# GenomicBreeding/GenomicBreedingModels.jl

Measured on AMD Instinct MI355X. Metric: GRM+GBLUP genotype-cells/s (n x p), higher is better.
Workload: dtype f64

## Files before the change

genomicbreedingmodels.jl_amd/csrc/capi.cpp:

```cpp
#include <cmath>

#include "fit_ctx.h"

namespace gbm {

static thread_local std::string g_last_error;

void set_error(const std::string& msg) { g_last_error = msg; }
int fail(int code, const std::string& msg) {
  g_last_error = msg;
  return code;
}
const std::string& last_error() { return g_last_error; }

int resolve_grm_mode(int grm_mode) {
  if (grm_mode != GBM_GRM_DEFAULT && grm_mode != GBM_GRM_DROPIN) return grm_mode;
  const char* e = ::gbm::knob("GBM_GRM");
  if (e && strcmp(e, "exact") == 0) return GBM_GRM_EXACT;
  if (e && strcmp(e, "auto") == 0) return GBM_GRM_AUTO;
  if (e && strcmp(e, "fp64") == 0) return GBM_GRM_FP64;
  return grm_mode == GBM_GRM_DROPIN ? GBM_GRM_AUTO : GBM_GRM_FP64;
}

namespace {

int solve_effects(const Problem& pr, Shards& shards, const std::vector<int>& leaders,
                  const std::vector<int>& ldevs, int64_t q, const double* Y, int64_t ldy, int64_t t0, int64_t nt,
                  double lambda, double* b_hat_out, double* y_pred_out, double* mu_out) {
  const int64_t n = pr.n, p = pr.p, npad = npad_of(n), gdim = gdim_of(n);
  const double inv_q = 1.0 / (double)q;
  const bool distributed = (leaders.size() > 1 || force_rccl()) && n >= knob_i64("GBM_DIST_SOLVE_MIN_N", 16384);
  std::vector<int32_t> infos(shards.size(), 0);
  {
    RoctxRange rsolve(distributed ? "gbm: distributed solve" : "gbm: solve");
    for (size_t k = 0; k < shards.size(); k++) {
      Shard& sh = *shards[k];
      FitCtx& c = sh.x();
      GBM_HIP_TRY(hipSetDevice(c.dev));
      hipStream_t s = c.stream.s;
      GBM_TRY(ensure(c.A, c.dev, nt * npad * 8));
      GBM_TRY(ensure(c.B, c.dev, nt * sh.p * 8));
      GBM_TRY(ensure(c.msum, c.dev, nt * 8));
      if (sh.leader != (int)k) continue;
      GBM_TRY(ensure(c.Y, c.dev, nt * npad * 8));
      GBM_TRY(ensure(c.gebv, c.dev, nt * npad * 8));
      GBM_TRY(ensure(c.mu, c.dev, nt * 8));
      GBM_TRY(ensure(c.info, c.dev, 4));
      const int64_t wss = gbm_dev_solve_workspace(n, nt);
      GBM_TRY(ensure(c.wss, c.dev, wss));
      GBM_HIP_TRY(hipMemcpy2DAsync(c.Y.p, npad * 8, Y + t0 * ldy, ldy * 8, n * 8, nt, hipMemcpyHostToDevice, s));
      if (!distributed)
        GBM_TRY(gbm_dev_gblup_solve((double*)c.G.p, gdim, n, inv_q, nullptr, lambda, (const double*)c.Y.p, npad, nt,
                                    (double*)c.A.p, (double*)c.gebv.p, npad, (double*)c.mu.p, (int32_t*)c.info.p,
                                    c.wss.p, wss, s));
    }
    if (distributed) GBM_TRY(solve_distributed(shards, leaders, ldevs, n, inv_q, lambda, nt));
    for (int k : leaders) {
      FitCtx& c = shards[k]->x();
      GBM_HIP_TRY(hipSetDevice(c.dev));
      GBM_HIP_TRY(hipMemcpyAsync(&infos[k], c.info.p, 4, hipMemcpyDeviceToHost, c.stream.s));
    }
    for (int k : leaders) {
      FitCtx& c = shards[k]->x();
      GBM_HIP_TRY(hipSetDevice(c.dev));
      GBM_HIP_TRY(hipStreamSynchronize(c.stream.s));
      const int32_t info = infos[k];
      if (info < 0) return fail(GBM_E_HIP, "solve: a wait between workgroups timed out (dataflow Cholesky or back substitution; the result is invalid)");
      if (info != 0)
        return fail(GBM_E_NOTPD, "G/q + lambda*I is not positive definite (pivot " + std::to_string(info) +
                                     "); check for non-finite genotypes");
    }
  }
  RoctxRange reff("gbm: marker effects + download");
  std::vector<std::vector<double>> msums(shards.size(), std::vector<double>(nt, 0.0));
  std::vector<double> mu(nt, 0.0);
  double* bo = b_hat_out + t0 * (p + 1);
  for (size_t k = 0; k < shards.size(); k++) {
    Shard& sh = *shards[k];
    FitCtx& c = sh.x();
    GBM_HIP_TRY(hipSetDevice(c.dev));
    hipStream_t s = c.stream.s;
    if (sh.leader != (int)k)
      GBM_HIP_TRY(hipMemcpyAsync(c.A.p, shards[sh.leader]->x().A.p, nt * npad * 8, hipMemcpyDeviceToDevice, s));
    if (sh.stream || sh.exact)
      GBM_TRY(stream_effects_shard(pr, sh, nt, inv_q));
    else
      GBM_TRY(gbm_dev_marker_effects((const double*)c.Xt.p, npad, sh.p, n, (const double*)c.A.p, npad, nt, inv_q,
                                     nullptr, (const double*)c.mean.p, (const double*)c.sd.p, (const int32_t*)c.keep.p,
                                     (double*)c.B.p, sh.p, (double*)c.msum.p, s));
    GBM_HIP_TRY(hipMemcpy2DAsync(bo + 1 + sh.j0, (p + 1) * 8, c.B.p, sh.p * 8, sh.p * 8, nt, hipMemcpyDeviceToHost, s));
    GBM_HIP_TRY(hipMemcpyAsync(msums[k].data(), c.msum.p, nt * 8, hipMemcpyDeviceToHost, s));
    if (k == 0) {
      GBM_HIP_TRY(hipMemcpy2DAsync(y_pred_out + t0 * n, n * 8, c.gebv.p, npad * 8, n * 8, nt, hipMemcpyDeviceToHost, s));
      GBM_HIP_TRY(hipMemcpyAsync(mu.data(), c.mu.p, nt * 8, hipMemcpyDeviceToHost, s));
    }
  }
  std::vector<double> msum_total(nt, 0.0);
  for (size_t k = 0; k < shards.size(); k++) {
    GBM_HIP_TRY(hipSetDevice(shards[k]->x().dev));
    GBM_HIP_TRY(hipStreamSynchronize(shards[k]->x().stream.s));
    for (int64_t t = 0; t < nt; t++) msum_total[t] += msums[k][t];
  }
  for (int64_t t = 0; t < nt; t++) {
    bo[t * (p + 1)] = mu[t] - msum_total[t];
    if (mu_out) mu_out[t0 + t] = mu[t];
  }
  return GBM_OK;
}

struct RemlOut {
  double* lambda;
  double* s2e;
  double* s2u;
};

int reml_lambda(FitCtx& c, int64_t n, int64_t q, const double* y, RemlResult& res) {
  const int64_t npad = npad_of(n), gdim = gdim_of(n);
  GBM_HIP_TRY(hipSetDevice(c.dev));
  hipStream_t s = c.stream.s;
  const int64_t wss = gbm_dev_solve_workspace(n, 1);
  GBM_TRY(ensure(c.Y, c.dev, npad * 8));
  GBM_TRY(ensure(c.A, c.dev, npad * 8));
  GBM_TRY(ensure(c.gebv, c.dev, npad * 8));
  GBM_TRY(ensure(c.mu, c.dev, 8));
  GBM_TRY(ensure(c.info, c.dev, 4));
  GBM_TRY(ensure(c.wss, c.dev, wss));
  GBM_TRY(ensure(c.tmp, c.dev, 4 * 8));
  const std::vector<double> ys = standardise_y(y, n);
  GBM_HIP_TRY(hipMemsetAsync(c.Y.p, 0, (size_t)(npad * 8), s));
  GBM_HIP_TRY(hipMemcpyAsync(c.Y.p, ys.data(), n * 8, hipMemcpyHostToDevice, s));
  auto eval = [&](double lambda, RemlEval& e) -> int {
    GBM_HIP_TRY(hipMemcpyAsync(c.G.p, c.Gc.p, (size_t)(npad * gdim * 8), hipMemcpyDeviceToDevice, s));
    GBM_TRY(gbm_dev_gblup_solve((double*)c.G.p, gdim, n, 1.0 / (double)q, nullptr, lambda, (const double*)c.Y.p, npad,
                                1, (double*)c.A.p, (double*)c.gebv.p, npad, (double*)c.mu.p, (int32_t*)c.info.p, c.wss.p,
                                wss, s));
    GBM_TRY(gbm_dev_gblup_terms((const double*)c.G.p, gdim, n, 1, c.wss.p, (double*)c.tmp.p, s));
    double t[4];
    int32_t info = 0;
    GBM_HIP_TRY(hipMemcpyAsync(t, c.tmp.p, 4 * 8, hipMemcpyDeviceToHost, s));
    GBM_HIP_TRY(hipMemcpyAsync(&info, c.info.p, 4, hipMemcpyDeviceToHost, s));
    GBM_HIP_TRY(hipStreamSynchronize(s));
    if (info < 0) return fail(GBM_E_HIP, "solve: a wait between workgroups timed out (dataflow Cholesky or back substitution; the result is invalid)");
    if (info != 0) return fail(GBM_E_NOTPD, "REML: G/q + lambda*I is not positive definite (pivot " + std::to_string(info) + ")");
    e = reml_profile(n, lambda, t);
    return GBM_OK;
  };
  return reml_search(eval, res);
}

int run_fit(const Problem& pr, const double* Y, int64_t ldy, int64_t nrhs, double lambda, const int* devices, int ndev,
            double* b_hat_out, double* y_pred_out, double* mu_out, int64_t* q_out, const RemlOut* reml = nullptr,
            int grm_mode = GBM_GRM_DEFAULT, int* grm_used_out = nullptr) {
  const int64_t n = pr.n, p = pr.p;
  if (n < 2) return fail(GBM_E_DATA, "there are less than 2 entries (reference src/prediction.jl:117-123)");
  if (p < 1 || pr.ld < n || !Y || ldy < n || nrhs < 1 || nrhs > 63 || !b_hat_out || !y_pred_out)
    return fail(GBM_E_ARG, "gbm_gblup_fit: bad arguments (need p >= 1, ldx >= n, ldy >= n, 1 <= nrhs <= 63, outputs)");
  if (!reml && (!(lambda > 0.0) || !std::isfinite(lambda)))
    return fail(GBM_E_ARG, "gbm_gblup_fit: lambda must be finite and > 0");
  if (reml && n < 3) return fail(GBM_E_DATA, "REML needs at least 3 entries");
  GBM_TRY(check_y(Y, n, ldy, nrhs));
  const int mode = resolve_grm_mode(grm_mode);
  if (mode != GBM_GRM_FP64 && mode != GBM_GRM_EXACT && mode != GBM_GRM_AUTO)
    return fail(GBM_E_ARG, "grm_mode must be GBM_GRM_DEFAULT, GBM_GRM_FP64, GBM_GRM_EXACT or GBM_GRM_AUTO (GBM_GRM: fp64 | exact | auto)");
  if (mode == GBM_GRM_EXACT && pr.src == Source::I8 && pr.ploidy != 2)
    return fail(GBM_E_ARG, "grm_mode exact: the exact-integer GRM needs diploid dosages (ploidy 2)");
  std::vector<int> devs;
  GBM_TRY(check_devices(devices, ndev, devs));
  const int64_t npad = npad_of(n), gdim = gdim_of(n);
  Shards shards;
  GBM_TRY(make_shards(devs, p, shards));
  int64_t q = 0, pmax = 0;
  for (auto& sh : shards) pmax = std::max(pmax, sh->p);
  const int64_t chunk = pr.src == Source::SYNTH ? 0 : host_chunk(pmax);
  bool exact = mode != GBM_GRM_FP64 && !(pr.src == Source::I8 && pr.ploidy != 2);
  const bool host_pack = knob_i64("GBM_HOST_PACK", 1) != 0;
  const int pack_threads = std::max(1, host_pack_threads() / (int)shards.size());
  auto fp64_grm = [&]() -> int {
    GBM_TRY(plan_streaming(pr, shards, reml != nullptr));
    const bool pack = mode == GBM_GRM_FP64 && pr.src == Source::F64 && host_pack;
    return parallel_shards(shards, [&](size_t, Shard& sh) {
      if (sh.stream) return stream_grm_shard(pr, sh);
      if (chunk > 0) {
        if (pack) {
          const int rc = upload_grm_pipelined_packed(pr, sh, chunk, pack_threads);
          if (rc != kNotDosage) return rc;
        }
        return upload_grm_pipelined(pr, sh, chunk);
      }
      return prepare_grm_shard(pr, sh);
    });
  };
  {
    RoctxRange r("gbm: upload + standardise + GRM");
    if (exact) {
      for (auto& sh : shards) sh->exact = true;
      const int rc = parallel_shards(shards, [&](size_t, Shard& sh) {
        if (pr.src == Source::F64) {
          if (host_pack)
            GBM_TRY(host_pack_upload_shard(pr, sh, pack_threads));
          else
            GBM_TRY(dosage_upload_shard(pr, sh, mode == GBM_GRM_AUTO));
        }
        return exact_grm_shard(pr, sh, mode == GBM_GRM_AUTO && pr.src == Source::I8);
      });
      if (rc == kNotDosage && mode == GBM_GRM_EXACT)
        return fail(GBM_E_ARG, "grm_mode exact: the genotypes are not diploid dosages (2x must be exactly 0, 1 or 2 "
                               "in every cell; use grm_mode auto or fp64)");
      const bool fallback = mode == GBM_GRM_AUTO && (rc == kNotDosage || rc == GBM_E_OOM || rc == GBM_E_ARG);
      if (fallback) {
        exact = false;
        for (auto& sh : shards) {
          sh->exact = sh->d8_ready = false;
          FitCtx& c = sh->x();
          if (pr.src == Source::F64 && c.D8.p) {
            (void)hipSetDevice(c.dev);
            c.D8.reset();
            c.D8.cap = 0;
          }
        }
        set_error("");
      } else {
        GBM_TRY(rc);
      }
    }
    if (!exact) GBM_TRY(fp64_grm());
  }
  if (grm_used_out) *grm_used_out = exact ? GBM_GRM_EXACT : GBM_GRM_FP64;
  for (auto& sh : shards) q += sh->q_host;
  if (q_out) *q_out = q;
  if (q == 0) return fail(GBM_E_DATA, "no polymorphic locus-allele (all standard deviations <= eps, src/gwas.jl:112-115)");
  {
    RoctxRange r("gbm: partial-GRM all-reduce");
    GBM_TRY(allreduce_grm(shards, n));
  }
  std::vector<int> leaders, ldevs;
  shard_leaders(shards, leaders, ldevs);
  if (!reml) return solve_effects(pr, shards, leaders, ldevs, q, Y, ldy, 0, nrhs, lambda, b_hat_out, y_pred_out, mu_out);
  const int64_t vbytes = npad * gdim * 8;
  FitCtx& c0 = shards[leaders[0]]->x();
  GBM_HIP_TRY(hipSetDevice(c0.dev));
  GBM_TRY(ensure(c0.Gc, c0.dev, gdim * gdim * 8));
  GBM_HIP_TRY(hipMemcpyAsync(c0.Gc.p, c0.G.p, (size_t)vbytes, hipMemcpyDeviceToDevice, c0.stream.s));
  std::vector<double> lam(nrhs);
  {
    RoctxRange r("gbm: REML lambda");
    for (int64_t t = 0; t < nrhs; t++) {
      RemlResult res;
      GBM_TRY(reml_lambda(shards[leaders[0]]->x(), n, q, Y + t * ldy, res));
      lam[t] = res.lambda;
      if (reml->lambda) reml->lambda[t] = res.lambda;
      if (reml->s2e) reml->s2e[t] = res.s2e;
      if (reml->s2u) reml->s2u[t] = res.s2u;
    }
  }
  GBM_HIP_TRY(hipSetDevice(c0.dev));
  GBM_HIP_TRY(hipStreamSynchronize(c0.stream.s));
  for (int64_t t = 0; t < nrhs; t++) {
    for (int k : leaders) {
      FitCtx& c = shards[k]->x();
      GBM_TRY(copy_dd(c, c.G.p, c0, c0.Gc.p, vbytes));
    }
    GBM_TRY(solve_effects(pr, shards, leaders, ldevs, q, Y, ldy, t, 1, lam[t], b_hat_out, y_pred_out, mu_out));
  }
  return GBM_OK;
}

int export_grm(FitCtx& c, int64_t n, double scale, double* G_out, int64_t ldg) {
  GBM_HIP_TRY(hipSetDevice(c.dev));
  GBM_TRY(ensure(c.out, c.dev, n * n * 8));
  GBM_TRY(launch_grm_export((const double*)c.G.p, gdim_of(n), n, scale, (double*)c.out.p, n, c.stream.s));
  GBM_HIP_TRY(hipMemcpy2DAsync(G_out, ldg * 8, c.out.p, n * 8, n * 8, n, hipMemcpyDeviceToHost, c.stream.s));
  GBM_HIP_TRY(hipStreamSynchronize(c.stream.s));
// ... 234 lines not shown
```

genomicbreedingmodels.jl_amd/csrc/chol.hip:

```cpp
#include <cstdlib>
#include <string>

#include "chol_device.h"

namespace gbm {

constexpr int NB = kCholNB;
constexpr int MAXRHS = 63;

int launch_chol_update(double* G, int64_t ldg, int64_t k0, int64_t nb, int64_t gdim, double* Ld, double* Dinv,
                       int32_t* info, int64_t next_k0, int rank, int nranks, hipStream_t s, int64_t col_lo = 0,
                       int64_t col_hi = INT64_MAX, int64_t row_lo = 0, int64_t row_hi = INT64_MAX);
int launch_chol_row_update(double* G, int64_t ldg, int64_t k0, int kch, int64_t gdim, double* Ld, double* Dinv,
                           int32_t* info, hipStream_t s, ColKeep keep = ColKeep{});
int64_t chol_small_lim();
void chol_refresh_tuning();
int64_t chol_flow_flag_bytes(int64_t gdim);
bool chol_flow_enabled(int64_t npad);
int launch_chol_flow(double* G, int64_t ldg, int64_t gdim, double* Ld, double* Dinv, void* flag_block, int32_t* info,
                     hipStream_t s);

__global__ void __launch_bounds__(256) prepare_v_kernel(double* __restrict__ G, int64_t ld, int64_t n,
                                                        int64_t npad, int64_t gdim, double inv_q,
                                                        const int64_t* __restrict__ q_dev, double lambda,
                                                        const double* __restrict__ Y, int64_t ldy, int64_t nrhs,
                                                        int32_t* __restrict__ info, ColKeep keep) {
  const int64_t i = blockIdx.x;
  if (i == 0 && threadIdx.x == 0) *info = 0;
  if (q_dev) inv_q = 1.0 / (double)(*q_dev);
  double* row = G + i * ld;
  const int64_t jbeg = (i / NB) * NB;
  for (int64_t j = jbeg + threadIdx.x; j < gdim; j += 256) {
    if (keep.nranks > 1 && !col_kept(keep, j)) continue;
    double v = 0.0;
    if (i < npad) {
      if (j < i) v = 0.0;
      else if (j < npad) v = (i < n && j < n) ? row[j] * inv_q + (i == j ? lambda : 0.0) : (i == j ? 1.0 : 0.0);
      else if (i < n) {
        const int64_t t = j - npad;
        v = t == 0 ? 1.0 : (t <= nrhs ? Y[(t - 1) * ldy + i] : 0.0);
      }
    }
    row[j] = v;
  }
}

__global__ void __launch_bounds__(256) factor_diag_kernel(const double* __restrict__ G, int64_t ld, int64_t k,
                                                          double* __restrict__ Ld, double* __restrict__ Dinv,
                                                          int32_t* __restrict__ info) {
  __shared__ __attribute__((aligned(16))) double Us[CNB * PS];
  __shared__ double rinv[CNB + 16];
  const int tid = threadIdx.x;
  {
    const int row = tid >> 2, quarter = tid & 3;
    const double* sa = G + (k + row) * ld + k + quarter * 16;
#pragma unroll
    for (int e = 0; e < 16; e += 2)
      *reinterpret_cast<double2*>(&Us[row * PS + quarter * 16 + e]) = *reinterpret_cast<const double2*>(sa + e);
  }
  __syncthreads();
  const int bad = factor_diag_block(Us, rinv, tid);
  if (tid == 0 && bad >= 0) atomicCAS(info, 0, (int32_t)(k + bad + 1));
  store_factor(Us, rinv, Ld + k * CNB, Dinv + (k / 16) * 256, tid);
}

__global__ void __launch_bounds__(256) chol_strip_kernel(double* __restrict__ G, int64_t ld, int64_t r0,
                                                         int64_t rows, int64_t J0, int64_t Jend, int64_t cnt,
                                                         int owner, int nranks, double* __restrict__ buf,
                                                         int unpack) {
  const int src = unpack ? (int)blockIdx.z : owner;
  const int64_t m = blockIdx.y;
  const int64_t row = (int64_t)blockIdx.x * 4 + (threadIdx.x >> 6);
  const int c2 = threadIdx.x & 63;
  if (row >= rows) return;
  const int64_t r = (m * rows + row) * 64 + c2;
  double2* b2 = reinterpret_cast<double2*>(buf) + (unpack ? (int64_t)src * cnt * rows * 64 + r : r);
  const int j0 = (int)J0;
  const int64_t J = J0 + ((src - j0) % nranks + nranks) % nranks + m * nranks;
  if (J >= Jend) {
    if (!unpack) *b2 = make_double2(0.0, 0.0);
    return;
  }
  double2* g2 = reinterpret_cast<double2*>(G + (r0 + row) * ld + J * 128) + c2;
  if (unpack)
    *g2 = *b2;
  else
    *b2 = *g2;
}

__global__ void __launch_bounds__(256) chol_panel_kernel(double* __restrict__ G, int64_t ld, int64_t k0,
                                                         const double* __restrict__ Ld,
                                                         const double* __restrict__ Dinv, ColKeep keep) {
  __shared__ __attribute__((aligned(16))) double Us[CNB * PS];
  __shared__ __attribute__((aligned(16))) double X[CNB * PS];
  __shared__ __attribute__((aligned(16))) double Di[4 * 256];
  const int tid = threadIdx.x, lane = tid & 63, wave = tid >> 6;
  const int64_t jx = k0 + ((int64_t)blockIdx.x + 1) * CNB;
  if (!col_kept(keep, jx)) return;
  const int lrow = tid >> 5, lcol = 2 * (tid & 31);
  {
    const double* sl = Ld + (k0 + lrow) * CNB + lcol;
    const double* sx = G + (k0 + lrow) * ld + jx + lcol;
    double2 vl[8], vx[8];
// ... 251 lines not shown
      *reinterpret_cast<double2*>(G + (jx + row) * ld + r0 + lcol) = make_double2(X[lcol * PS + row], X[(lcol + 1) * PS + row]);
    }
    if (area) {
#pragma unroll
      for (int ks = 0; ks < 16; ks++) {
        double af[2], bf[2];
#pragma unroll
        for (int m = 0; m < 2; m++) af[m] = -X[(ks * 4 + fr) * PS + wm * 32 + m * 16 + fc];
#pragma unroll
        for (int q = 0; q < 2; q++) bf[q] = X[(ks * 4 + fr) * PS + wn * 32 + q * 16 + fc];
#pragma unroll
        for (int m = 0; m < 2; m++)
#pragma unroll
          for (int q = 0; q < 2; q++) accd[m][q] = __builtin_amdgcn_mfma_f64_16x16x4f64(af[m], bf[q], accd[m][q], 0, 0, 0);
      }
      publish_flag(&prog[c], j + 1, tid);
    } else {
      __syncthreads();
    }
  }
}

__global__ void __launch_bounds__(64) diag_inverse_kernel(const double* __restrict__ Ld, double* __restrict__ Linv) {
  __shared__ double Ub[NB][NB + 1];
  const int lane = threadIdx.x;
  const int64_t b0 = (int64_t)blockIdx.x * NB;
  for (int r = 0; r < NB; r++) Ub[r][lane] = Ld[(b0 + r) * NB + lane];
  __syncthreads();
  double x[NB];
#pragma unroll
  for (int i = NB - 1; i >= 0; i--) {
    double p0 = 0.0, p1 = 0.0, p2 = 0.0, p3 = 0.0;
#pragma unroll
    for (int k = i + 1; k < NB; k += 4) {
      p0 = fma(Ub[i][k], x[k], p0);
      if (k + 1 < NB) p1 = fma(Ub[i][k + 1], x[k + 1], p1);
      if (k + 2 < NB) p2 = fma(Ub[i][k + 2], x[k + 2], p2);
      if (k + 3 < NB) p3 = fma(Ub[i][k + 3], x[k + 3], p3);
    }
    x[i] = (i <= lane) ? (((lane == i) ? 1.0 : 0.0) - ((p0 + p1) + (p2 + p3))) * rcp_nr(Ub[i][i]) : 0.0;
  }
#pragma unroll
  for (int i = 0; i < NB; i++) Linv[(b0 + i) * NB + lane] = x[i];
}

__global__ void __launch_bounds__(256) gls_mu_kernel(const double* __restrict__ G, int64_t ld, int64_t npad,
                                                     int64_t nrhs, double* __restrict__ W, int64_t lda,
                                                     double* __restrict__ mu, int32_t* __restrict__ flags) {
  const int64_t t = blockIdx.y;
  const double c11 = -G[npad * ld + npad];
  const double c1y = -G[npad * ld + npad + 1 + t];
  const double m = c1y / c11;
  if (blockIdx.x == 0 && threadIdx.x == 0) mu[t] = m;
  if (t == 0)
    for (int64_t i = (int64_t)blockIdx.x * 256 + threadIdx.x; i < npad / NB; i += (int64_t)gridDim.x * 256) flags[i] = 0;
  for (int64_t i = (int64_t)blockIdx.x * 256 + threadIdx.x; i < lda; i += (int64_t)gridDim.x * 256)
    W[t * lda + i] = i < npad ? G[(npad + 1 + t) * ld + i] - m * G[npad * ld + i] : 0.0;
}

__global__ void __launch_bounds__(256) gblup_terms_kernel(const double* __restrict__ G, int64_t ld, int64_t npad,
                                                          int64_t nrhs, const double* __restrict__ Ld,
                                                          double* __restrict__ terms) {
  __shared__ double red[256];
  double sacc = 0.0;
  for (int64_t r = threadIdx.x; r < npad; r += 256) sacc += log(Ld[r * NB + (r % NB)]);
  red[threadIdx.x] = sacc;
  __syncthreads();
  for (int w = 128; w > 0; w >>= 1) {
    if ((int)threadIdx.x < w) red[threadIdx.x] += red[threadIdx.x + w];
    __syncthreads();
  }
  if (threadIdx.x == 0) {
    terms[0] = 2.0 * red[0];
    terms[1] = -G[npad * ld + npad];
  }
  for (int64_t t = threadIdx.x; t < nrhs; t += 256) {
    terms[2 + 2 * t] = -G[npad * ld + npad + 1 + t];
    terms[3 + 2 * t] = -G[(npad + 1 + t) * ld + npad + 1 + t];
  }
}

constexpr int RC = 4;

__global__ void __launch_bounds__(256) back_solve_kernel(const double* __restrict__ G, int64_t ld,
                                                         const double* __restrict__ Linv, int64_t nb,
                                                         const double* __restrict__ W, double* A,
                                                         int64_t lda, int64_t nrhs, int32_t* __restrict__ flags,
                                                         int32_t* __restrict__ info) {
  __shared__ double part[4][RC][NB];
  __shared__ double rl[RC][NB];
  __shared__ double ah[RC][NB];
  __shared__ int ok_s;
  const int tid = threadIdx.x, lane = tid & 63, wave = tid >> 6;
  const int64_t bh = nb - 1 - 2 * (int64_t)blockIdx.x, bl = bh - 1;
  const bool lo = bl >= 0;
  const int64_t h0 = bh * NB, l0 = bl * NB;
  const int j0 = wave * 16;
  const int64_t a_bytes = nrhs * lda * 8;
  const __amdgpu_buffer_rsrc_t rA =
      __builtin_amdgcn_make_buffer_rsrc(A, (short)0, (int)(a_bytes < 0x7fffffff ? a_bytes : 0x7fffffff), 0x00020000);
  double uh[16], ul[16], lb[16];
#pragma unroll
  for (int jj = 0; jj < 16; jj++) {
    uh[jj] = Linv[(h0 + lane) * NB + j0 + jj];
    ul[jj] = lo ? Linv[(l0 + lane) * NB + j0 + jj] : 0.0;
    lb[jj] = lo ? G[(h0 + j0 + jj) * ld + l0 + lane] : 0.0;
  }
  if (tid == 0) ok_s = 1;
  int32_t pass = 0;
  auto solve_block = [&](int64_t b0, const double (&ui)[16], const double (&acc)[RC], const double (&w)[RC], int tc,
                         int64_t t0, double (*out)[NB]) {
#pragma unroll
    for (int t = 0; t < RC; t++) part[wave][t][lane] = acc[t];
    lds_sync();
    if (wave == 0)
#pragma unroll
      for (int t = 0; t < RC; t++)
        if (t < tc) rl[t][lane] = w[t] - (((part[0][t][lane] + part[1][t][lane]) + part[2][t][lane]) + part[3][t][lane]);
    lds_sync();
    for (int t = 0; t < tc; t++) {
      double s = 0.0;
#pragma unroll
      for (int jj = 0; jj < 16; jj++) s = fma(ui[jj], rl[t][j0 + jj], s);
      part[wave][t][lane] = s;
    }
    lds_sync();
    if (wave == 0)
      for (int t = 0; t < tc; t++) {
        const double v = ((part[0][t][lane] + part[1][t][lane]) + part[2][t][lane]) + part[3][t][lane];
        st_agent(A + (t0 + t) * lda + b0 + lane, v);
        if (out) out[t][lane] = v;
      }
  };
  for (int64_t t0 = 0; t0 < nrhs; t0 += RC) {
    pass++;
    const int tc = (int)(nrhs - t0 < RC ? nrhs - t0 : RC);
    double acch[RC] = {0.0, 0.0, 0.0, 0.0}, accl[RC] = {0.0, 0.0, 0.0, 0.0};
    double wh[RC] = {0.0, 0.0, 0.0, 0.0}, wl[RC] = {0.0, 0.0, 0.0, 0.0};
    if (wave == 0)
#pragma unroll
      for (int t = 0; t < RC; t++)
        if (t < tc) {
          wh[t] = W[(t0 + t) * lda + h0 + lane];
          if (lo) wl[t] = W[(t0 + t) * lda + l0 + lane];
        }
    bool ok = true;
    for (int64_t c = nb - 1; c > bh && ok; c--) {
      double lh[16], ll[16];
      const double* lp = G + (c * NB + j0) * ld + lane;
#pragma unroll
      for (int jj = 0; jj < 16; jj++) {
        lh[jj] = lp[(int64_t)jj * ld + h0];
        ll[jj] = lo ? lp[(int64_t)jj * ld + l0] : 0.0;
      }
      if (lane == 0) ok = wait_flag<false>(&flags[c], pass, info);
      ok = __builtin_amdgcn_readfirstlane((int)ok) != 0;
      __builtin_amdgcn_fence(__ATOMIC_ACQUIRE, "wavefront");
      for (int t = 0; t < tc; t++) {
        const uint32_t voff = (uint32_t)(((t0 + t) * lda + c * NB + j0) * 8);
        double av[16];
#pragma unroll
        for (int jj = 0; jj < 16; jj++)
          av[jj] = __builtin_bit_cast(double, __builtin_amdgcn_raw_buffer_load_b64(rA, (int)(voff + jj * 8), 0, 16));
        double sh = 0.0, sl = 0.0;
#pragma unroll
        for (int jj = 0; jj < 16; jj++) {
          sh = fma(lh[jj], av[jj], sh);
          sl = fma(ll[jj], av[jj], sl);
        }
        acch[t] += sh;
        accl[t] += sl;
      }
    }
    if (!ok) ok_s = 0;
    solve_block(h0, uh, acch, wh, tc, t0, lo ? ah : nullptr);
    publish_flag(&flags[bh], pass, tid);
    if (lo) {
      for (int t = 0; t < tc; t++) {
        double sl = 0.0;
#pragma unroll
        for (int jj = 0; jj < 16; jj++) sl = fma(lb[jj], ah[t][j0 + jj], sl);
        accl[t] += sl;
      }
      lds_sync();
      solve_block(l0, ul, accl, wl, tc, t0, nullptr);
      publish_flag(&flags[bl], pass, tid);
    }
    if (!ok_s) return;
    lds_sync();
  }
}

constexpr int WPA = CNB + 4;
__global__ void __launch_bounds__(512) whiten_rows_kernel(const double* __restrict__ G, int64_t ldg,
                                                          const double* __restrict__ Linv, int64_t nb, double* R,
                                                          int64_t ldr, int64_t rows) {
  __shared__ __attribute__((aligned(16))) double As[2][CNB * WPA];
  __shared__ __attribute__((aligned(16))) double Bs[2][CNB * PS];
  const int tid = threadIdx.x, lane = tid & 63, wave = tid >> 6;
  const int wm = wave >> 2, wn = wave & 3, fr = lane >> 4, fc = lane & 15;
  const int64_t r0 = (int64_t)blockIdx.x * CNB;
  const int lrow = tid >> 5, lcol = 2 * (tid & 31);
  const int cw = wn * 16 + fc;
  typedef double d8 __attribute__((ext_vector_type(8)));
  for (int64_t k = 0; k < nb; k++) {
    d4 acc[2];
#pragma unroll
    for (int m = 0; m < 2; m++)
#pragma unroll
      for (int r = 0; r < 4; r++) {
        const int64_t row = r0 + wm * 32 + m * 16 + fr + 4 * r;
        acc[m][r] = row < rows ? R[row * ldr + k * CNB + cw] : 0.0;
      }
    d8 va0, vb0, va1, vb1;
    auto load_step = [&](int64_t m, d8& va, d8& vb) {
#pragma unroll
      for (int e = 0; e < 4; e++) {
        const int64_t row = r0 + lrow + 16 * e;
        double2 x = make_double2(0.0, 0.0);
        if (row < rows) x = *reinterpret_cast<const double2*>(R + row * ldr + m * CNB + lcol);
        const double2 y = *reinterpret_cast<const double2*>(G + (m * CNB + lrow + 16 * e) * ldg + k * CNB + lcol);
        va[2 * e] = x.x;
        va[2 * e + 1] = x.y;
        vb[2 * e] = y.x;
        vb[2 * e + 1] = y.y;
      }
    };
    auto stage = [&](int buf, const d8& va, const d8& vb) {
#pragma unroll
      for (int e = 0; e < 4; e++) {
        *reinterpret_cast<double2*>(&As[buf][(lrow + 16 * e) * WPA + lcol]) = make_double2(va[2 * e], va[2 * e + 1]);
        *reinterpret_cast<double2*>(&Bs[buf][(lrow + 16 * e) * PS + lcol]) = make_double2(vb[2 * e], vb[2 * e + 1]);
      }
    };
    auto step = [&](int64_t m, int buf, d8& na, d8& nb_) {
      const double* Am = As[buf];
      const double* Bm = Bs[buf];
#pragma unroll
      for (int ks = 0; ks < 16; ks++) {
        const double bf = Bm[(ks * 4 + fr) * PS + cw];
#pragma unroll
        for (int mm = 0; mm < 2; mm++) {
          const double af = -Am[(wm * 32 + mm * 16 + fc) * WPA + ks * 4 + fr];
          acc[mm] = __builtin_amdgcn_mfma_f64_16x16x4f64(af, bf, acc[mm], 0, 0, 0);
        }
      }
      if (m + 1 < k) {
        stage(buf ^ 1, na, nb_);
        if (m + 3 < k) load_step(m + 3, na, nb_);
      }
      __syncthreads();
    };
    if (k > 0) {
      load_step(0, va0, vb0);
      if (k > 1) load_step(1, va1, vb1);
      stage(0, va0, vb0);
      if (k > 2) load_step(2, va0, vb0);
      __syncthreads();
    }
    for (int64_t m = 0; m < k; m += 2) {
      step(m, 0, va1, vb1);
      if (m + 1 < k) step(m + 1, 1, va0, vb0);
    }
#pragma unroll
    for (int m = 0; m < 2; m++)
#pragma unroll
      for (int r = 0; r < 4; r++) As[0][(wm * 32 + m * 16 + fr + 4 * r) * WPA + cw] = acc[m][r];
#pragma unroll
// ... 18 lines not shown
#pragma unroll
      for (int r = 0; r < 4; r++) {
        const int64_t row = r0 + wm * 32 + m * 16 + fr + 4 * r;
        if (row < rows) R[row * ldr + k * CNB + cw] = out[m][r];
      }
    __builtin_amdgcn_s_waitcnt(0);
    __syncthreads();
  }
}

__global__ void __launch_bounds__(256) gebv_kernel(const double* __restrict__ Y, int64_t ldy, int64_t n,
                                                   const double* __restrict__ A, double* __restrict__ gebv,
                                                   int64_t lda, const double* __restrict__ mu, double lambda) {
  const int64_t t = blockIdx.y;
  const double m = mu[t];
  for (int64_t i = (int64_t)blockIdx.x * 256 + threadIdx.x; i < lda; i += (int64_t)gridDim.x * 256)
    gebv[t * lda + i] = i < n ? m + (Y[t * ldy + i] - m) - lambda * A[t * lda + i] : 0.0;
}

}

using namespace gbm;

extern "C" int64_t gbm_dev_npad(int64_t n) { return npad_of(n); }
extern "C" int64_t gbm_dev_gdim(int64_t n) { return gdim_of(n); }
static int64_t flow_block_offset(int64_t n) { return round_up(npad_of(n) * (2 * NB + 16) + npad_of(n) / NB / 2 + 1, 2); }
static int64_t solve_ws_doubles(int64_t n) { return flow_block_offset(n) + chol_flow_flag_bytes(gdim_of(n)) / 8; }
extern "C" int64_t gbm_dev_solve_workspace(int64_t n, int64_t nrhs) {
  (void)nrhs;
  return solve_ws_doubles(n) * (int64_t)sizeof(double);
}

namespace {

struct SolveWs {
  double *Ld, *Linv, *Dinv;
  int32_t* flags;
  void* flow;
};
SolveWs solve_ws(void* workspace, int64_t npad) {
  SolveWs w;
  w.Ld = (double*)workspace;
  w.Linv = w.Ld + npad * NB;
  w.Dinv = w.Linv + npad * NB;
  w.flags = reinterpret_cast<int32_t*>(w.Dinv + npad * 16);
  w.flow = (double*)workspace + flow_block_offset(npad);
  return w;
}

int check_solve_args(const double* G, int64_t ldg, int64_t n, const int32_t* info, const void* workspace,
                     int64_t ws_bytes, const char* who) {
  if (!G || !info || n < 1 || ldg < gdim_of(n) || (ldg & 1) || ((uintptr_t)G & 15))
    return fail(GBM_E_ARG, std::string(who) + ": bad arguments (G 16-byte aligned, even ldg >= gdim(n))");
  if (!workspace || ws_bytes < solve_ws_doubles(n) * (int64_t)sizeof(double) || ((uintptr_t)workspace & 15))
    return fail(GBM_E_ARG, std::string(who) + ": workspace too small (see gbm_dev_solve_workspace)");
  return GBM_OK;
}

static int64_t tail_flow_rows(int64_t npad) {
  const char* e = ::gbm::knob("GBM_CHOL_TAIL_FLOW");
  if (e) return (int64_t)atoll(e);
  return npad > 12288 ? 8192 : 0;
}
static bool tail_flow_at(int64_t kb, int64_t npad, int64_t gdim) {
  return kb > 0 && kb < npad / NB && gdim - kb * NB <= tail_flow_rows(npad);
}

int group_size(int64_t kb, int64_t nb, int64_t gdim) {
  if (tail_flow_at(kb, nb * NB, gdim)) return (int)(nb - kb);
  auto lim = [](const char* name, int64_t dflt) {
    const char* e = ::gbm::knob(name);
    return e ? (int64_t)atoll(e) : dflt;
  };
  const int64_t g4 = lim("GBM_CHOL_G4_LIM", 8192), g8 = lim("GBM_CHOL_G8_LIM", 8192),
                g16 = lim("GBM_CHOL_G16_LIM", 16384);
  const int64_t k0 = kb * NB;
  if (g16 >= 0 && kb + 16 < nb && gdim - (k0 + 16 * NB) > g16) return 16;
  if (g8 >= 0 && kb + 8 < nb && gdim - (k0 + 8 * NB) > g8) return 8;
  if (g4 >= 0 && kb + 4 < nb && gdim - (k0 + 4 * NB) > g4) return 4;
  if (kb + 2 < nb && gdim - (k0 + 2 * NB) > chol_small_lim()) return 2;
  return 1;
}

int solve_prepare(double* G, int64_t ldg, int64_t n, double inv_q, const int64_t* q_dev, double lambda,
                  const double* Y, int64_t ldy, int64_t nrhs, int32_t* info, void* workspace, hipStream_t s,
                  bool factor_first = true, ColKeep keep = ColKeep{}) {
  const int64_t npad = npad_of(n), gdim = gdim_of(n);
  const SolveWs w = solve_ws(workspace, npad);
  chol_refresh_tuning();
  prepare_v_kernel<<<(unsigned)gdim, 256, 0, s>>>(G, ldg, n, npad, gdim, inv_q, q_dev, lambda, Y, ldy, nrhs, info,
                                                  keep);
  GBM_LAUNCH_CHECK();
  if (!factor_first) return GBM_OK;
  factor_diag_kernel<<<1, 256, 0, s>>>(G, ldg, 0, w.Ld, w.Dinv, info);
  GBM_LAUNCH_CHECK();
  return GBM_OK;
}

static bool group_kernel_enabled() {
  const char* e = ::gbm::knob("GBM_CHOL_GROUP_KERNEL");
  return !e || atoi(e) != 0;
}

int solve_group_panels(double* G, int64_t ldg, int64_t n, int64_t kb, ColKeep keep, int32_t* info, void* workspace,
                       hipStream_t s, int64_t* g_out) {
  const int64_t npad = npad_of(n), gdim = gdim_of(n), nb = npad / NB;
  const SolveWs w = solve_ws(workspace, npad);
  const int64_t k0 = kb * NB;
  if (tail_flow_at(kb, npad, gdim))
    return fail(GBM_E_ARG, "gbm_dev_chol_group_panels: the dataflow tail (GBM_CHOL_TAIL_FLOW) runs as gbm_dev_chol_group");
  const int g = group_size(kb, nb, gdim);
  if (keep.nranks > 1) {
    if (g < 2 || (k0 % 128) != 0)
      return fail(GBM_E_ARG, "gbm_dev_chol_group_panels: a distributed step needs a panel group of >= 2 panels on a "
                             "128-row boundary (finish the tail with gbm_dev_chol_group, nranks = 1)");
    keep.keep_hi = k0 + g * NB;
    keep.rhs0 = npad;
  }
  if (g_out) *g_out = g;
  if (g > 1 && group_kernel_enabled()) {
    GroupCols gc;
    gc.g = g;
    gc.nranks = keep.nranks;
    gc.a0 = kb + g;
    gc.rhs0 = npad / NB;
    gc.n_rhs = (gdim - npad) / NB;
    if (keep.nranks == 1) {
      gc.n_own = npad / NB - gc.a0;
    } else {
      const int64_t R = keep.nranks, J0 = gc.a0 / 2;
      if ((gc.a0 & 1) != 0) return fail(GBM_E_ARG, "gbm_dev_chol_group_panels: odd panel group in a distributed step");
      gc.J_first = J0 + ((keep.rank - J0) % R + R) % R;
      for (int64_t J = gc.J_first; 2 * J < npad / NB; J += R) gc.n_own += (2 * J + 1 < npad / NB) ? 2 : 1;
    }
    if ((int64_t)(CNB + 1) * ldg * 8 > 0x7fffffff)
      return fail(GBM_E_ARG, "chol_group_kernel: ldg too large for 32-bit buffer offsets");
    int32_t* prog = reinterpret_cast<int32_t*>(w.flow);
    GBM_HIP_TRY(hipMemsetAsync(prog, 0, (size_t)g * sizeof(int32_t), s));
    const int64_t nwg = (g - 1) + gc.n_own + gc.n_rhs;
    chol_group_kernel<<<(unsigned)nwg, 256, 0, s>>>(G, ldg, k0, gc, w.Ld, w.Dinv, prog, info);
    GBM_LAUNCH_CHECK();
    return GBM_OK;
  }
  auto panel = [&](int64_t k) {
    const int64_t chunks = (gdim - k) / NB - 1;
    chol_panel_kernel<<<(unsigned)chunks, 256, 0, s>>>(G, ldg, k, w.Ld, w.Dinv, keep);
    return hipGetLastError() == hipSuccess;
  };
  if (!panel(k0)) return fail(GBM_E_HIP, "chol_panel_kernel launch failed");
  for (int j = 1; j < g; j++) {
    GBM_TRY(launch_chol_row_update(G, ldg, k0, j, gdim, w.Ld, w.Dinv, info, s, keep));
    if (!panel(k0 + j * NB)) return fail(GBM_E_HIP, "chol_panel_kernel launch failed");
  }
  return GBM_OK;
}

int solve_group_update(double* G, int64_t ldg, int64_t n, int64_t kb, int rank, int nranks, int32_t* info,
                       void* workspace, hipStream_t s, int64_t col_lo = 0, int64_t col_hi = INT64_MAX,
                       int64_t row_lo = 0, int64_t row_hi = INT64_MAX) {
  const int64_t npad = npad_of(n), gdim = gdim_of(n), nb = npad / NB;
  const SolveWs w = solve_ws(workspace, npad);
  const int64_t k0 = kb * NB;
  if (tail_flow_at(kb, npad, gdim))
    return fail(GBM_E_ARG, "gbm_dev_chol_group_update: the dataflow tail (GBM_CHOL_TAIL_FLOW) runs as gbm_dev_chol_group");
  const int g = group_size(kb, nb, gdim);
  const int64_t next = kb + g < nb ? k0 + g * NB : -1;
  if (g > 1)
    return launch_chol_update(G, ldg, k0, g * NB, gdim, w.Ld, w.Dinv, info, next, rank, nranks, s, col_lo, col_hi,
                              row_lo, row_hi);
  if (nranks > 1) return fail(GBM_E_ARG, "gbm_dev_chol_group_update: single-panel steps are not distributed");
  return launch_chol_update(G, ldg, k0, NB, gdim, w.Ld, w.Dinv, info, next, 0, 1, s);
}

int solve_group(double* G, int64_t ldg, int64_t n, int64_t kb, int32_t* info, void* workspace, hipStream_t s,
                int64_t* g_out) {
  const int64_t npad = npad_of(n), gdim = gdim_of(n);
  if (tail_flow_at(kb, npad, gdim)) {
    const SolveWs w = solve_ws(workspace, npad);
    const int64_t k0 = kb * NB;
    if (g_out) *g_out = npad / NB - kb;
    return launch_chol_flow(G + k0 * ldg + k0, ldg, gdim - k0, w.Ld + k0 * CNB, w.Dinv + (k0 / 16) * 256, w.flow,
                            info, s);
  }
  GBM_TRY(solve_group_panels(G, ldg, n, kb, ColKeep{}, info, workspace, s, g_out));
  return solve_group_update(G, ldg, n, kb, 0, 1, info, workspace, s);
}

int solve_finish(double* G, int64_t ldg, int64_t n, const double* Y, int64_t ldy, int64_t nrhs, double lambda,
                 double* A_out, double* gebv, int64_t lda, double* mu, int32_t* info, void* workspace, hipStream_t s) {
  const int64_t npad = npad_of(n), nb = npad / NB;
  const SolveWs w = solve_ws(workspace, npad);
  diag_inverse_kernel<<<(unsigned)nb, 64, 0, s>>>(w.Ld, w.Linv);
  GBM_LAUNCH_CHECK();
  const unsigned gx = (unsigned)((lda + 255) / 256 < 1024 ? (lda + 255) / 256 : 1024);
  gls_mu_kernel<<<dim3(gx, (unsigned)nrhs), 256, 0, s>>>(G, ldg, npad, nrhs, gebv, lda, mu, w.flags);
  GBM_LAUNCH_CHECK();
  back_solve_kernel<<<(unsigned)((nb + 1) / 2), 256, 0, s>>>(G, ldg, w.Linv, nb, gebv, A_out, lda, nrhs, w.flags, info);
  GBM_LAUNCH_CHECK();
  gebv_kernel<<<dim3(gx, (unsigned)nrhs), 256, 0, s>>>(Y, ldy, n, A_out, gebv, lda, mu, lambda);
  GBM_LAUNCH_CHECK();
  return GBM_OK;
}

void strip_geometry(int64_t n, int64_t kb, int64_t rows64, int nranks, int64_t& r0, int64_t& rows, int64_t& J0,
                    int64_t& Jend, int64_t& cnt, bool area = false) {
  r0 = kb * NB;
  rows = rows64 * NB;
  J0 = r0 / 128;
  Jend = area ? (r0 + rows + 127) / 128 : npad_of(n) / 128;
  cnt = Jend > J0 ? (Jend - J0 + nranks - 1) / nranks : 0;
}

}

extern "C" int gbm_dev_gblup_solve(double* G, int64_t ldg, int64_t n, double inv_q, const int64_t* q_dev,
                                   double lambda, const double* Y, int64_t ldy, int64_t nrhs, double* A_out,
                                   double* gebv, int64_t lda, double* mu, int32_t* info, void* workspace,
                                   int64_t ws_bytes, void* stream) {
  const int64_t npad = npad_of(n);
  if (!Y || !A_out || !gebv || !mu || ldy < n || lda < npad || nrhs < 1 || nrhs > MAXRHS || !(lambda > 0.0) ||
      !(q_dev || inv_q > 0.0))
    return fail(GBM_E_ARG, "gbm_dev_gblup_solve: bad arguments (need ldg >= gdim(n), lda >= npad(n), "
                           "1 <= nrhs <= 63, lambda > 0, inv_q > 0)");
  GBM_TRY(check_solve_args(G, ldg, n, info, workspace, ws_bytes, "gbm_dev_gblup_solve"));
  hipStream_t s = (hipStream_t)stream;
  if (chol_flow_enabled(npad)) {
    GBM_TRY(solve_prepare(G, ldg, n, inv_q, q_dev, lambda, Y, ldy, nrhs, info, workspace, s, false));
    const SolveWs w = solve_ws(workspace, npad);
    GBM_TRY(launch_chol_flow(G, ldg, gdim_of(n), w.Ld, w.Dinv, w.flow, info, s));
    return solve_finish(G, ldg, n, Y, ldy, nrhs, lambda, A_out, gebv, lda, mu, info, workspace, s);
  }
  GBM_TRY(solve_prepare(G, ldg, n, inv_q, q_dev, lambda, Y, ldy, nrhs, info, workspace, s));
  const int64_t nb = npad / NB;
  for (int64_t kb = 0; kb < nb;) {
    int64_t g = 1;
    GBM_TRY(solve_group(G, ldg, n, kb, info, workspace, s, &g));
    kb += g;
  }
  return solve_finish(G, ldg, n, Y, ldy, nrhs, lambda, A_out, gebv, lda, mu, info, workspace, s);
}

extern "C" int gbm_dev_chol_prepare(double* G, int64_t ldg, int64_t n, double inv_q, const int64_t* q_dev,
                                    double lambda, const double* Y, int64_t ldy, int64_t nrhs, int32_t* info,
                                    void* workspace, int64_t ws_bytes, void* stream) {
  if (!Y || ldy < n || nrhs < 1 || nrhs > MAXRHS || !(lambda > 0.0) || !(q_dev || inv_q > 0.0))
    return fail(GBM_E_ARG, "gbm_dev_chol_prepare: bad arguments");
  GBM_TRY(check_solve_args(G, ldg, n, info, workspace, ws_bytes, "gbm_dev_chol_prepare"));
  return solve_prepare(G, ldg, n, inv_q, q_dev, lambda, Y, ldy, nrhs, info, workspace, (hipStream_t)stream);
}

extern "C" int gbm_dev_chol_prepare_cols(double* G, int64_t ldg, int64_t n, double inv_q, const int64_t* q_dev,
                                         double lambda, const double* Y, int64_t ldy, int64_t nrhs, int rank,
                                         int nranks, int32_t* info, void* workspace, int64_t ws_bytes, void* stream) {
  if (!Y || ldy < n || nrhs < 1 || nrhs > MAXRHS || !(lambda > 0.0) || !(q_dev || inv_q > 0.0) || nranks < 1 ||
      rank < 0 || rank >= nranks)
    return fail(GBM_E_ARG, "gbm_dev_chol_prepare_cols: bad arguments");
  GBM_TRY(check_solve_args(G, ldg, n, info, workspace, ws_bytes, "gbm_dev_chol_prepare_cols"));
  ColKeep keep;
  keep.rank = rank;
  keep.nranks = nranks;
  if (nranks > 1) {
    chol_refresh_tuning();
    keep.keep_hi = (int64_t)group_size(0, npad_of(n) / NB, gdim_of(n)) * NB;
    keep.rhs0 = npad_of(n);
  }
  return solve_prepare(G, ldg, n, inv_q, q_dev, lambda, Y, ldy, nrhs, info, workspace, (hipStream_t)stream, true, keep);
}

extern "C" int64_t gbm_dev_chol_group_size(int64_t n, int64_t kb) {
  const int64_t nb = npad_of(n) / NB;
  if (kb < 0 || kb >= nb) return 0;
  chol_refresh_tuning();
  return group_size(kb, nb, gdim_of(n));
}

extern "C" int gbm_dev_chol_group(double* G, int64_t ldg, int64_t n, int64_t kb, int rank, int nranks, int32_t* info,
                                  void* workspace, int64_t ws_bytes, void* stream) {
  GBM_TRY(check_solve_args(G, ldg, n, info, workspace, ws_bytes, "gbm_dev_chol_group"));
  if (kb < 0 || kb >= npad_of(n) / NB || nranks != 1 || rank != 0)
    return fail(GBM_E_ARG, "gbm_dev_chol_group: one rank only (rank 0 of 1); a distributed step is "
                           "gbm_dev_chol_group_panels + row exchange + gbm_dev_chol_group_update");
  return solve_group(G, ldg, n, kb, info, workspace, (hipStream_t)stream, nullptr);
}

extern "C" int gbm_dev_chol_group_panels(double* G, int64_t ldg, int64_t n, int64_t kb, int rank, int nranks,
                                         int32_t* info, void* workspace, int64_t ws_bytes, void* stream) {
  GBM_TRY(check_solve_args(G, ldg, n, info, workspace, ws_bytes, "gbm_dev_chol_group_panels"));
  if (kb < 0 || kb >= npad_of(n) / NB || nranks < 1 || rank < 0 || rank >= nranks)
    return fail(GBM_E_ARG, "gbm_dev_chol_group_panels: bad step or rank");
  ColKeep keep;
  keep.rank = rank;
  keep.nranks = nranks;
  return solve_group_panels(G, ldg, n, kb, keep, info, workspace, (hipStream_t)stream, nullptr);
}

extern "C" int gbm_dev_chol_group_update(double* G, int64_t ldg, int64_t n, int64_t kb, int rank, int nranks,
                                         int32_t* info, void* workspace, int64_t ws_bytes, void* stream) {
  GBM_TRY(check_solve_args(G, ldg, n, info, workspace, ws_bytes, "gbm_dev_chol_group_update"));
  if (kb < 0 || kb >= npad_of(n) / NB || nranks < 1 || rank < 0 || rank >= nranks)
    return fail(GBM_E_ARG, "gbm_dev_chol_group_update: bad step or rank");
  return solve_group_update(G, ldg, n, kb, rank, nranks, info, workspace, (hipStream_t)stream);
}

extern "C" int gbm_dev_chol_group_update_cols(double* G, int64_t ldg, int64_t n, int64_t kb, int rank, int nranks,
                                              int64_t col_lo, int64_t col_hi, int32_t* info, void* workspace,
                                              int64_t ws_bytes, void* stream) {
  GBM_TRY(check_solve_args(G, ldg, n, info, workspace, ws_bytes, "gbm_dev_chol_group_update_cols"));
  if (kb < 0 || kb >= npad_of(n) / NB || nranks < 2 || rank < 0 || rank >= nranks || col_lo < 0 || col_hi < col_lo)
    return fail(GBM_E_ARG, "gbm_dev_chol_group_update_cols: bad step, rank (nranks >= 2) or column range");
  return solve_group_update(G, ldg, n, kb, rank, nranks, info, workspace, (hipStream_t)stream, col_lo, col_hi);
}

extern "C" int gbm_dev_chol_group_update_tiles(double* G, int64_t ldg, int64_t n, int64_t kb, int rank, int nranks,
                                               int64_t row_lo, int64_t row_hi, int64_t col_lo, int64_t col_hi,
                                               int32_t* info, void* workspace, int64_t ws_bytes, void* stream) {
  GBM_TRY(check_solve_args(G, ldg, n, info, workspace, ws_bytes, "gbm_dev_chol_group_update_tiles"));
  if (kb < 0 || kb >= npad_of(n) / NB || nranks < 2 || rank < 0 || rank >= nranks || col_lo < 0 || col_hi < col_lo ||
      row_lo < 0 || row_hi < row_lo)
    return fail(GBM_E_ARG, "gbm_dev_chol_group_update_tiles: bad step, rank (nranks >= 2), row or column range");
  return solve_group_update(G, ldg, n, kb, rank, nranks, info, workspace, (hipStream_t)stream, col_lo, col_hi, row_lo,
                            row_hi);
}
// ... 125 lines not shown
```

genomicbreedingmodels.jl_amd/csrc/chol_flow.hip:

```cpp
#include <atomic>
#include <cstdlib>
#include <map>
#include <mutex>
#include <type_traits>
#include <vector>

#include "chol_device.h"

namespace gbm {

namespace {

typedef double dbl2 __attribute__((ext_vector_type(2)));
typedef unsigned int u4 __attribute__((ext_vector_type(4)));
typedef unsigned int u2 __attribute__((ext_vector_type(2)));
constexpr int FT = 64;
constexpr int32_t kPairBit = 0x8000;
constexpr int kTraceRec = 32;
constexpr int kSc1 = 16;

__device__ __forceinline__ __amdgpu_buffer_rsrc_t rsrc(const void* p, int64_t bytes) {
  return __builtin_amdgcn_make_buffer_rsrc(const_cast<void*>(p), (short)0, (int)bytes, 0x00020000);
}
__device__ __forceinline__ dbl2 ld2(__amdgpu_buffer_rsrc_t r, uint32_t voff, uint32_t soff) {
// ... 830 lines not shown
  return o;
}

int flow_order_variant() {
  const char* ev = ::gbm::knob("GBM_CHOL_FLOW_ORDER");
  const int v = ev ? atoi(ev) : 5;
  return v == 4 || v == 6 ? v : 5;
}

std::vector<int32_t> flow_order(int nbc) { return flow_order(nbc, flow_order_variant()); }

int64_t flow_order_check(int nbc, const int32_t* order, int64_t m) {
  const int nb = nbc - 1;
  std::vector<int64_t> pos((size_t)nbc * nbc, -1);
  int64_t tiles = 0;
  for (int64_t t = 0; t < m; t++) {
    const int i = order[t] >> 16, j = order[t] & 0x7fff, nt = (order[t] & kPairBit) ? 2 : 1;
    if (i < 0 || j < i || j + nt - 1 > nb || (i == 0 && j == 0) || (nt == 2 && j < i + 2)) return t + 1;
    for (int q = 0; q < nt; q++) {
      if (pos[(size_t)i * nbc + j + q] >= 0) return t + 1;
      pos[(size_t)i * nbc + j + q] = t;
      tiles++;
    }
  }
  if (tiles != (int64_t)nbc * (nbc + 1) / 2 - 1) return m + 1;
  auto at = [&](int i, int j) { return pos[(size_t)i * nbc + j]; };
  std::vector<int64_t> chain_need(nbc, -1);
  for (int s = 0; s < nb; s++) {
    int64_t need = s > 0 ? chain_need[s - 1] : -1;
    need = std::max(need, at(s, s + 1));
    if (s + 1 < nb) need = std::max(need, at(s + 1, s + 1));
    if (s >= 1) need = std::max(need, at(s - 1, s + 1));
    chain_need[s] = need;
  }
  for (int64_t t = 0; t < m; t++) {
    const int i = order[t] >> 16, nt = (order[t] & kPairBit) ? 2 : 1;
    for (int j = order[t] & 0x7fff, q = 0; q < nt; q++, j++) {
      const bool diag = i == j, nbr = j == i + 1;
      const int kend = ((diag && i < nb) || (nbr && i >= 1)) ? i - 1 : i;
      for (int k = 0; k < kend; k++)
        if (at(k, i) > t || at(k, j) > t || chain_need[k] > t) return t + 1;
      if (!diag && !nbr && chain_need[i] > t) return t + 1;
    }
  }
  return 0;
}

namespace {

int flow_order_dev(int nbc, const int32_t** out, int* count) {
  static std::mutex mu;
  static auto* cache = new std::map<std::pair<int, int>, std::pair<int32_t*, int>>;
  int dev = 0;
  GBM_HIP_TRY(hipGetDevice(&dev));
  const int variant = flow_order_variant();
  std::lock_guard<std::mutex> lock(mu);
  auto it = cache->find({dev, nbc * 8 + variant});
  if (it == cache->end()) {
    const std::vector<int32_t> o = flow_order(nbc, variant);
    int32_t* d = nullptr;
    GBM_HIP_TRY(hipMalloc((void**)&d, o.size() * sizeof(int32_t)));
    GBM_HIP_TRY(hipMemcpy(d, o.data(), o.size() * sizeof(int32_t), hipMemcpyHostToDevice));
    it = cache->emplace(std::make_pair(dev, nbc * 8 + variant), std::make_pair(d, (int)o.size())).first;
  }
  *out = it->second.first;
  *count = it->second.second;
  return GBM_OK;
}

}

int64_t chol_flow_flag_bytes(int64_t gdim) {
  const int64_t nbc = gdim / FT;
  return round_up(16 + nbc * nbc * 4, 16);
}

bool chol_flow_enabled(int64_t npad) {
  const char* e = ::gbm::knob("GBM_CHOL_FLOW_MAX");
  const int64_t lim = e ? (int64_t)atoll(e) : (int64_t)12288;
  return npad <= lim;
}

int launch_chol_flow(double* G, int64_t ldg, int64_t gdim, double* Ld, double* Dinv, void* flag_block, int32_t* info,
                     hipStream_t s) {
  const int64_t nbc = gdim / FT;
  const int64_t ntasks = nbc * (nbc + 1) / 2;
  if (nbc < 2 || (int64_t)FT * ldg * 8 > 0x7fffffff || nbc * nbc > 0x3fffffff || nbc > 0x7fff)
    return fail(GBM_E_ARG, "dataflow Cholesky: matrix too large for 32-bit buffer offsets");
  const int32_t* order = nullptr;
  int nwork = 0;
  GBM_TRY(flow_order_dev((int)nbc, &order, &nwork));
  GBM_HIP_TRY(hipMemsetAsync(flag_block, 0, (size_t)chol_flow_flag_bytes(gdim), s));
  if (::gbm::knob("GBM_TEST_CHOL_FLOW_ABORT")) GBM_HIP_TRY(hipMemsetAsync(info, 0xFF, sizeof(int32_t), s));
  const char* ew = ::gbm::knob("GBM_CHOL_FLOW_WGS");
  const int64_t workers = ew && atoll(ew) > 0 ? atoll(ew) : flow_cus() - 2;
  const unsigned grid = (unsigned)(2 + (nwork < workers ? nwork : (workers < 1 ? 1 : workers)));
  int32_t* q = (int32_t*)flag_block;
  const char* ex = ::gbm::knob("GBM_CHOL_FLOW_XN");
  const int xn_defer = ex && atoi(ex) == 0 ? 0 : 1;
  if (::gbm::knob("GBM_CHOL_FLOW_TRACE")) {
    const int64_t nrec = ntasks + nbc;
    if (g_trace_cap < nrec) {
      if (g_trace) (void)hipFree(g_trace);
      g_trace = nullptr;
      GBM_HIP_TRY(hipMalloc((void**)&g_trace, (size_t)nrec * kTraceRec * 8));
      g_trace_cap = nrec;
    }
    GBM_HIP_TRY(hipMemsetAsync(g_trace, 0, (size_t)nrec * kTraceRec * 8, s));
    g_trace_n = nrec;
    const int tm = atoi(::gbm::knob("GBM_CHOL_FLOW_TRACE"));
    const int roles = tm > 1 ? (tm & 7) : 7;
    if (::gbm::knob("GBM_CHOL_FLOW_TRACE_PLAIN"))
      chol_flow_kernel<false><<<grid, 256, 0, s>>>(G, ldg, (int)nbc, Ld, Dinv, q, q + 4, info, order, nwork, xn_defer, nullptr, 0);
    else
    chol_flow_kernel<true><<<grid, 256, 0, s>>>(G, ldg, (int)nbc, Ld, Dinv, q, q + 4, info, order, nwork, xn_defer, g_trace, roles);
  } else {
    chol_flow_kernel<false><<<grid, 256, 0, s>>>(G, ldg, (int)nbc, Ld, Dinv, q, q + 4, info, order, nwork, xn_defer, nullptr, 0);
  }
  GBM_LAUNCH_CHECK();
  return GBM_OK;
}

}

extern "C" int64_t gbm_debug_chol_flow_trace(int64_t* host, int64_t cap) {
  using namespace gbm;
  if (!g_trace || !host) return 0;
  const int64_t n = g_trace_n < cap ? g_trace_n : cap;
  if (hipDeviceSynchronize() != hipSuccess || hipMemcpy(host, g_trace, (size_t)n * kTraceRec * 8, hipMemcpyDeviceToHost) != hipSuccess)
    return -1;
  return n;
}

extern "C" int64_t gbm_debug_chol_flow_order(int nbc, int32_t* order_out, int64_t cap) {
  if (nbc < 2 || nbc > 0x7fff) return -1;
  const std::vector<int32_t> o = gbm::flow_order(nbc);
  if (order_out && cap >= (int64_t)o.size()) std::copy(o.begin(), o.end(), order_out);
  return gbm::flow_order_check(nbc, o.data(), (int64_t)o.size());
}

extern "C" int64_t gbm_debug_chol_flow_order_size(int nbc) {
  if (nbc < 2 || nbc > 0x7fff) return -1;
  return (int64_t)gbm::flow_order(nbc).size();
}

extern "C" int64_t gbm_debug_chol_flow_order_check(int nbc, const int32_t* order, int64_t m) {
  if (nbc < 2 || nbc > 0x7fff || !order) return -1;
  return gbm::flow_order_check(nbc, order, m);
}
```

genomicbreedingmodels.jl_amd/csrc/fit_ctx.h:

```cpp
#pragma once
#include <algorithm>
#include <cstring>
#include <map>
#include <memory>
#include <mutex>
#include <string>
#include <thread>
#include <vector>

#include "gbm_internal.h"
#include "host_util.h"

namespace gbm {


struct FitCtx {
  int dev = 0;
  Stream stream;
  Stream copy;
  std::vector<hipEvent_t> ev;
  DevBuf Xt, D8, mean, sd, keep, q, G, Gc, wsg, Y, A, gebv, mu, info, wss, B, msum, packed, out, part;
  DevBuf tmp, strip, gathered;
  DevBuf errs, q2;
  DevBuf astrip, agathered;
  hipEvent_t ev_area = nullptr, ev_upd = nullptr;
  HostPinned pack;
  ~FitCtx() {
    (void)hipSetDevice(dev);
    for (hipEvent_t e : ev) (void)hipEventDestroy(e);
    if (ev_area) (void)hipEventDestroy(ev_area);
    if (ev_upd) (void)hipEventDestroy(ev_upd);
  }
};

inline CtxPool<FitCtx>& pool() { return CtxPool<FitCtx>::instance(); }

struct Shard {
  std::unique_ptr<FitCtx> c;
  int64_t j0 = 0, p = 0, q_host = 0;
  int64_t stream = 0;
  bool exact = false;
  bool d8_ready = false;
  int leader = -1;
  ~Shard() {
    if (c) pool().release(std::move(c));
  }
  FitCtx& x() { return *c; }
};
using Shards = std::vector<std::unique_ptr<Shard>>;

enum class Source { F64, I8, SYNTH };

struct Problem {
  Source src;
  const double* X;
  const int8_t* D;
  int ploidy;
  int64_t n, p, ld;
  uint64_t seed = 0;
};

constexpr int kNotDosage = 1;

inline bool each_shard_leads() {
  const char* e = ::gbm::knob("GBM_SHARD_LEADERS");
  return e && strcmp(e, "each") == 0;
}

inline int make_shards(const std::vector<int>& devs, int64_t p, Shards& shards) {
  const int nd = (int)std::min<int64_t>((int64_t)devs.size(), p);
  const int64_t per = (p + nd - 1) / nd;
  const bool each = each_shard_leads();
  for (int k = 0; k < nd; k++) {
    const int64_t j0 = k * per;
    if (j0 >= p) break;
    auto sh = std::make_unique<Shard>();
    GBM_TRY(pool().acquire(devs[k], sh->c));
    sh->j0 = j0;
    sh->p = std::min(per, p - j0);
    for (size_t m = 0; m < shards.size() && !each; m++)
      if (shards[m]->x().dev == devs[k]) {
        sh->leader = shards[m]->leader;
        break;
      }
    if (sh->leader < 0) sh->leader = (int)shards.size();
    shards.push_back(std::move(sh));
  }
  return GBM_OK;
}

inline void shard_leaders(Shards& shards, std::vector<int>& leaders, std::vector<int>& ldevs) {
  for (size_t k = 0; k < shards.size(); k++)
    if (shards[k]->leader == (int)k) {
      leaders.push_back((int)k);
      ldevs.push_back(shards[k]->x().dev);
    }
}

template <class Fn>
int parallel_shards(Shards& shards, Fn&& fn) {
  const size_t m = shards.size();
  const char* e = ::gbm::knob("GBM_SHARD_THREADS");
  if (m == 1 || (e && strcmp(e, "0") == 0)) {
    for (size_t k = 0; k < m; k++) GBM_TRY(fn(k, *shards[k]));
    return GBM_OK;
  }
  std::vector<int> rc(m, GBM_OK);
  std::vector<std::string> msg(m);
  auto run = [&](size_t k) {
    rc[k] = fn(k, *shards[k]);
    if (rc[k] != GBM_OK) msg[k] = last_error();
  };
  std::vector<std::thread> th;
  th.reserve(m - 1);
  for (size_t k = 1; k < m; k++) {
    try {
      th.emplace_back(run, k);
    } catch (...) {
      run(k);
    }
  }
  run(0);
  for (auto& t : th) t.join();
  for (size_t k = 0; k < m; k++)
    if (rc[k] < 0) return fail(rc[k], msg[k]);
  for (size_t k = 0; k < m; k++)
    if (rc[k] != GBM_OK) return fail(rc[k], msg[k]);
  return GBM_OK;
}

int ensure_copy_stream(FitCtx& c);
int64_t host_chunk(int64_t p);
int prepare_shard(const Problem& pr, Shard& sh, bool center_only = false, bool sync = true);
int grm_shard(const Problem& pr, Shard& sh);
int prepare_grm_shard(const Problem& pr, Shard& sh);
int upload_grm_pipelined(const Problem& pr, Shard& sh, int64_t chunk);
int upload_grm_pipelined_packed(const Problem& pr, Shard& sh, int64_t chunk, int threads);
int plan_streaming(const Problem& pr, Shards& shards, bool reml);
int stream_grm_shard(const Problem& pr, Shard& sh);
int dosage_upload_shard(const Problem& pr, Shard& sh, bool early_exit);
int host_pack_upload_shard(const Problem& pr, Shard& sh, int threads);
int exact_grm_shard(const Problem& pr, Shard& sh, bool check_bytes = false);
int stream_effects_shard(const Problem& pr, Shard& sh, int64_t nt, double inv_q);

int copy_dd(FitCtx& dst, void* d, const FitCtx& src, const void* s, int64_t bytes, hipStream_t on = nullptr);
bool force_rccl();
int allreduce_grm(Shards& shards, int64_t n);
int solve_distributed(Shards& shards, const std::vector<int>& leaders, const std::vector<int>& ldevs, int64_t n,
                      double inv_q, double lambda, int64_t nrhs);
void rccl_call_counts(int64_t* allreduce, int64_t* allgather);

}
```

genomicbreedingmodels.jl_amd/csrc/gbm_internal.h:

```cpp
#pragma once
#include <hip/hip_runtime.h>
#include <stdint.h>
#include <functional>
#include <string>
#include <vector>

#include "../../include/gbm.h"

namespace gbm {

constexpr int64_t kNPadTile = 128;
constexpr int64_t kRhsRows = 64;
constexpr int kCholNB = 64;

inline int64_t round_up(int64_t x, int64_t m) { return (x + m - 1) / m * m; }
inline int64_t npad_of(int64_t n) { return round_up(n < 1 ? 1 : n, kNPadTile); }
inline int64_t gdim_of(int64_t n) { return npad_of(n) + kRhsRows; }

void set_error(const std::string& msg);
int fail(int code, const std::string& msg);
const std::string& last_error();

const char* knob(const char* name);
int64_t knob_i64(const char* name, int64_t def);

#define GBM_HIP_TRY(expr)                                                                      \
  do {                                                                                         \
    hipError_t e_ = (expr);                                                                    \
    if (e_ != hipSuccess)                                                                      \
      return ::gbm::fail(GBM_E_HIP, std::string("HIP error '") + hipGetErrorString(e_) +       \
                                        "' at " __FILE__ ":" + std::to_string(__LINE__) + " (" #expr ")"); \
  } while (0)

#define GBM_LAUNCH_CHECK() GBM_HIP_TRY(hipGetLastError())

#define GBM_TRY(expr)              \
  do {                             \
    int rc_ = (expr);              \
    if (rc_ != GBM_OK) return rc_; \
  } while (0)

int launch_grm(const double* Zt, int64_t ldz, int64_t p, int64_t n, double* G, int64_t ldg,
               void* ws, int64_t ws_bytes, hipStream_t s, int accum = 0, int32_t* err_out = nullptr);
bool grm_can_accumulate(int64_t n, int64_t p);
int launch_standardize_rows(const double* Xt, int64_t ldx, int64_t p, int64_t n, double* Zt, int64_t ldz, double* mean,
                            double* sd, int32_t* keep, int64_t* q_dev, hipStream_t s, bool beside_tiles = false);
bool standardize_fits_beside_tiles(int64_t n);
int64_t grm_workspace_bytes(int64_t n, int64_t p);
int launch_grm_export(const double* G, int64_t ldg, int64_t n, double inv_q, double* out, int64_t ldo, hipStream_t s);
int launch_predict(const double* Xt, int64_t ldx, int64_t p, int64_t n, const double* b, int64_t ldb, int64_t nrhs,
                   double* partial, int64_t nchunks, double* out, int64_t ldo, hipStream_t s);
int64_t predict_chunks(int64_t n, int64_t p);
int launch_add_inplace(double* a, const double* b, int64_t n, hipStream_t s);
int launch_standardize_i8(const int8_t* D, int64_t ldd, int64_t p, int64_t n, int ploidy, double* Zt, int64_t ldz,
                          double* mean, double* sd, int32_t* keep, int64_t* q_dev, hipStream_t s);
int launch_marker_rows(const double* Zt, int64_t ldz, int64_t p, int64_t n, const double* A, int64_t lda, int64_t nrhs,
                       double inv_q, const int64_t* q_dev, const double* sd, const int32_t* keep, double* B,
                       int64_t ldb, hipStream_t s);
int launch_marker_rows_i8(const int8_t* D, int64_t ldd, int64_t p, int64_t n, int ploidy, const double* A, int64_t lda,
                          int64_t nrhs, double inv_q, const int64_t* q_dev, const double* mean, const double* sd,
                          const int32_t* keep, double* B, int64_t ldb, hipStream_t s);
int launch_grm_exact(const int8_t* D, int64_t ldd, int64_t p, int64_t n, int ploidy, double* G, int64_t ldg,
                     double* mean, double* sd, int32_t* keep, int64_t* q_dev, int accum, void* ws, int64_t ws_bytes,
                     int32_t* slices_out, hipStream_t s);
int grm_exact_status(const void* ws, int64_t n, int64_t p, hipStream_t s);
int launch_gather_dosage(const double* Xt, int64_t ldx, int64_t p, const int32_t* idx, int64_t nT, int8_t* D,
                         hipStream_t s);
int launch_dosage_from_f64(const double* X, int64_t ldx, int64_t n, int64_t p, int8_t* D, int64_t ldd, int32_t* bad,
                           hipStream_t s);
int launch_dosage_check_i8(const int8_t* D, int64_t ldd, int64_t n, int64_t p, int32_t* bad, hipStream_t s);
bool pack_dosage_columns(const double* X, int64_t ld, int64_t n, int64_t p, int8_t* dst);
int host_pack_threads();
class ChunkPacker {
 public:
  ChunkPacker(const double* X, int64_t ld, int64_t n, const std::vector<std::pair<int64_t, int64_t>>& sched,
              int8_t* ring, int64_t slot_bytes, int slots, int threads);
  ~ChunkPacker();
  ChunkPacker(const ChunkPacker&) = delete;
  ChunkPacker& operator=(const ChunkPacker&) = delete;
  const int8_t* wait(int64_t k);
  void release_upto(int64_t k);

 private:
  struct Impl;
  Impl* d_;
};
int resolve_grm_mode(int grm_mode);
int launch_weighted_sum(const double* mean, const double* B, int64_t ldb, int64_t p, int64_t nrhs, double* msum,
                        hipStream_t s);
struct GwasCoef {
  double Ainv[64];
  double Au[8];
  double zscale;
  int32_t kcov;
};
int launch_gwas_stats(const double* W, int64_t ldw, int64_t rows, int64_t n, const double* Cw, int64_t ldcw,
                      const double* yw, const GwasCoef& co, const int32_t* keep, double* z, double* b, double* s_out,
                      unsigned long long* tested, hipStream_t s);
int launch_center_columns(const double* Xt, int64_t ldx, int64_t p, int64_t n, double* Zt, int64_t ldz, double* mean,
                          double* sd, int32_t* keep, int64_t* q_dev, hipStream_t s);

int64_t enet_lda(int64_t n);
int launch_enet_x2(const double* Z, int64_t ldz, int64_t p, int64_t n, double* x2, hipStream_t s);
int launch_enet_gather(const double* Z, int64_t ldz, int64_t n, const int32_t* rows, int64_t a0, int64_t cnt,
                       const double* x2, double* Za, int64_t lda, double* x2a, hipStream_t s);
int64_t enet_gram_workspace(int64_t n);
int launch_enet_gram(const double* Za, int64_t lda, int64_t A, int64_t n, int64_t blk0, double* W, double* ws,
                     hipStream_t s);
int launch_enet_prep(int64_t A, const double* x2a, double l2, double* invden, hipStream_t s);
int launch_enet_pass(const double* Za, int64_t lda, int64_t n, int64_t A, const double* W, const double* x2a,
                     const double* invden, const double* b_in, double* b_out, double thr, double* partial,
                     double* blkmax, double* e, double* red, hipStream_t s);
int launch_enet_norm(const double* e, int64_t n, double* red, hipStream_t s);

constexpr int kPcsBlock = 32;
int64_t rows_times_sym_splits(int64_t n);
int launch_pcs_colstats(const double* K, int64_t ldk, int64_t n, double* m, double* s, hipStream_t st);
int launch_pcs_rowtrace(const double* K, int64_t ldk, int64_t n, const double* m, const double* s, double* rows_out,
                        hipStream_t st);
int launch_pcs_sum(const double* x, int64_t stride, int64_t n, double* out, hipStream_t st);
int launch_pcs_ref_mid(const double* Qt, int64_t ldq, const double* P, int64_t ldp, int64_t n, const double* m,
                       const double* s, double* Wt, int64_t ldw, hipStream_t st);
int launch_pcs_ref_post(const double* Wt, int64_t ldw, int64_t n, const double* m, double* Yt, int64_t ldy,
                        hipStream_t st);
int64_t pcs_gram_workspace(int64_t n);
int launch_pcs_gram(const double* A, int64_t lda, const double* B, int64_t ldb, int64_t n, int npairs, double* part,
                    double* out, hipStream_t st);
// ... 33 lines not shown
```

genomicbreedingmodels.jl_amd/csrc/grm.hip:

```cpp
#include <algorithm>
#include <atomic>
#include <cmath>
#include <cstdio>
#include <cstdlib>
#include <map>
#include <mutex>
#include <queue>
#include <tuple>
#include <vector>

#include "chol_device.h"

namespace gbm {

constexpr int BT = 128;
constexpr int BK = 16;
constexpr int WPS = 2;
constexpr int LROW = BT + 2;
constexpr int STAGE = 2 * BK * LROW;

__device__ __forceinline__ void tile_of(int64_t t, int64_t& ti, int64_t& tj) {
  int64_t r = (int64_t)((sqrt(8.0 * (double)t + 1.0) - 1.0) * 0.5);
  while ((r + 1) * (r + 2) / 2 <= t) r++;
  while (r * (r + 1) / 2 > t) r--;
// ... 434 lines not shown
    }
    const bool diag = (ti == tj);
    const int64_t i0 = c0 + ti * BT, j0 = c0 + tj * BT;
    const bool active = (i0 + wm * 64 < rlim) && (j0 + wn * 64 < rlim) && !(diag && wm == 1 && wn == 0);
    d4 acc[4][4];
    const int64_t col0 = j0 + wn * 64 + 4 * frag_col;
#pragma unroll
    for (int m = 0; m < 4; m++)
#pragma unroll
      for (int r = 0; r < 4; r++) {
        const int64_t row = i0 + wm * 64 + 4 * frag_row + 16 * r + m;
        double2 c01 = make_double2(0.0, 0.0), c23 = make_double2(0.0, 0.0);
        if (active && row < rlim && col0 < rlim) {
          c01 = *reinterpret_cast<const double2*>(C + row * ldc + col0);
          c23 = *reinterpret_cast<const double2*>(C + row * ldc + col0 + 2);
        }
        acc[m][0][r] = c01.x;
        acc[m][1][r] = c01.y;
        acc[m][2][r] = c23.x;
        acc[m][3][r] = c23.y;
      }
    tile_pass<true>(U, ldu, K, i0, j0, diag, active, 0, nst, lds, acc, wave, lane);
    const bool factor_next = fk0 >= 0 && wg == 0;
    if (!active && !factor_next) return;
#pragma unroll
    for (int m = 0; m < 4; m++)
#pragma unroll
      for (int r = 0; r < 4; r++) {
        const int64_t row = i0 + wm * 64 + 4 * frag_row + 16 * r + m;
        if (active && row < rlim && col0 < rlim) {
          *reinterpret_cast<double2*>(C + row * ldc + col0) = make_double2(acc[m][0][r], acc[m][1][r]);
          *reinterpret_cast<double2*>(C + row * ldc + col0 + 2) = make_double2(acc[m][2][r], acc[m][3][r]);
        }
      }
    if (factor_next) {
      double* Us = lds;
      double* rinv = lds + CNB * PS;
      if (wave == 0) {
#pragma unroll
        for (int m = 0; m < 4; m++)
#pragma unroll
          for (int q = 0; q < 4; q++)
#pragma unroll
            for (int r = 0; r < 4; r++) Us[(4 * frag_row + 16 * r + m) * PS + 4 * frag_col + q] = acc[m][q][r];
      }
      __syncthreads();
      const int bad = factor_diag_block(Us, rinv, threadIdx.x);
      if (threadIdx.x == 0 && bad >= 0) atomicCAS(info, 0, (int32_t)(fk0 + bad + 1));
      store_factor(Us, rinv, Ld + fk0 * CNB, Dinv + (fk0 / 16) * 256, threadIdx.x);
    }
  }
}

#ifndef GBM_GRM_RED_NT
#define GBM_GRM_RED_NT 1
#endif
__global__ void __launch_bounds__(256) grm_slab_reduce_kernel(const double* __restrict__ slab, int64_t ntiles,
                                                              int nslices, double* __restrict__ G, int64_t ldg,
                                                              int accum) {
  const int64_t t = blockIdx.x;
  int64_t ti, tj;
  tile_of(t, ti, tj);
  const int64_t per = (int64_t)BT * BT;
  for (int e = threadIdx.x * 2; e < BT * BT; e += 256 * 2) {
    double2 acc = make_double2(0.0, 0.0);
    for (int sl = 0; sl < nslices; sl++) {
#if GBM_GRM_RED_NT
      typedef double d2v __attribute__((ext_vector_type(2)));
      const d2v v = __builtin_nontemporal_load(reinterpret_cast<const d2v*>(slab + ((int64_t)sl * ntiles + t) * per + e));
#else
      const double2 v = *reinterpret_cast<const double2*>(slab + ((int64_t)sl * ntiles + t) * per + e);
#endif
      acc.x += v.x;
      acc.y += v.y;
    }
    const int row = e / BT, col = e % BT;
    double2* g = reinterpret_cast<double2*>(G + (ti * BT + row) * ldg + tj * BT + col);
    if (accum) {
      const double2 old = *g;
      acc.x = old.x + acc.x;
      acc.y = old.y + acc.y;
    }
    *g = acc;
  }
}

static int resident_wgs() {
  int dev = 0, cus = 256;
  if (hipGetDevice(&dev) == hipSuccess) {
    int v = 0;
    if (hipDeviceGetAttribute(&v, hipDeviceAttributeMultiprocessorCount, dev) == hipSuccess && v > 0) cus = v;
  }
  return cus * WPS;
}

struct GrmTuning {
  int carry = -1;
  bool edge = true;
  bool persist = true;
  bool edge_concurrent = true;
  bool fuse = false;
  bool diag = true;
  double diag_cost = 0.66;
  std::vector<double> split;
};

static GrmTuning grm_tuning() {
  GrmTuning t;
  auto flag = [](const char* name, bool dflt) {
    const char* e = ::gbm::knob(name);
    return e ? atoi(e) != 0 : dflt;
  };
  if (const char* e = ::gbm::knob("GBM_GRM_CARRY")) t.carry = atoi(e) != 0 ? 1 : 0;
  t.edge = flag("GBM_GRM_EDGE", true);
  t.persist = flag("GBM_GRM_PERSIST", true);
  t.edge_concurrent = flag("GBM_GRM_EDGE_CONCURRENT", true);
  t.fuse = flag("GBM_GRM_FUSED", false);
  t.diag = flag("GBM_GRM_DIAG", true);
  if (const char* e = ::gbm::knob("GBM_GRM_DIAG_COST")) {
    const double c = atof(e);
    if (c > 0.0 && c <= 1.0) t.diag_cost = c;
  }
  if (!t.diag) t.diag_cost = 0.93;
  if (const char* ov = ::gbm::knob("GBM_GRM_SPLIT")) {
    for (const char* q = ov; *q;) {
      char* end = nullptr;
      const double x = strtod(q, &end);
      if (end == q) break;
      if (x > 0) t.split.push_back(x);
      q = (*end == ',') ? end + 1 : end;
    }
    if ((int)t.split.size() > kMaxSlices) t.split.clear();
  }
  return t;
}

struct GrmPlan {
  int64_t ntiles, nst, tile_elems;
  SliceBounds sb;
  int64_t main_doubles, edge_doubles;
  bool persist, edge_concurrent;
};

static double simulate_split(const std::vector<int64_t>& sizes, const std::vector<double>& cost, int64_t R,
                             double tile_bytes, double stage_s, bool carry) {
  std::vector<double> speed(R);
  uint64_t h = 0x9E3779B97F4A7C15ull;
  for (int64_t k = 0; k < R; k++) {
    h = h * 6364136223846793005ull + 1442695040888963407ull;
    speed[k] = 1.0 + 0.035 * (((double)(h >> 11) / 9007199254740992.0) * 2.0 - 1.0);
  }
  std::priority_queue<std::pair<double, int64_t>, std::vector<std::pair<double, int64_t>>, std::greater<>> slots;
  for (int64_t k = 0; k < R; k++) slots.push({0.0, k});
  double makespan = 0.0;
  for (size_t s = 0; s < sizes.size(); s++)
    for (double c : cost) {
      auto [f, k] = slots.top();
      slots.pop();
      f += (double)sizes[s] * c * ((s == 0 && f > 0.0) ? 1.10 : 1.0) / speed[k];
      if (carry && s > 0) f += 0.5;
      if (f > makespan) makespan = f;
      slots.push({f, k});
    }
  const double reduce_stages =
      carry ? 0.0 : (double)sizes.size() * (double)cost.size() * tile_bytes / 4e12 / stage_s;
  return makespan + reduce_stages;
// ... 411 lines not shown
                                             nullptr, -1, TileOwner{});
    GBM_LAUNCH_CHECK();
  }
  if (g.sb.er > 0) {
    rc = launch_grm_edge(g, Zt, ldz, p, n, G, ldg, ws, accum, ax ? ax->s : s);
    if (rc != GBM_OK) return rc;
    if (ax) {
      GBM_HIP_TRY(hipEventRecord(ax->join, ax->s));
      GBM_HIP_TRY(hipStreamWaitEvent(s, ax->join, 0));
    }
  }
  return GBM_OK;
}

int launch_standardize_grm_syrk(const double* X, int64_t ldx, int64_t p, int64_t n, double* Zt, int64_t ldz,
                                double* mean, double* sd, int32_t* keep, int64_t* q, double* G, int64_t ldg, void* ws,
                                int64_t ws_bytes, hipStream_t s) {
  int rc = check_grm_args(Zt, ldz, p, n, G, ldg);
  if (rc != GBM_OK) return rc;
  if (!X || !mean || !sd || !keep || !q || ldx < n || (X == Zt && ldx != ldz))
    return fail(GBM_E_ARG, "gbm_dev_standardize_grm_syrk: bad arguments");
  const GrmPlan g = plan(n, p);
  const int64_t h = g.sb.n >= 2 ? std::min<int64_t>(p, (int64_t)BK * g.sb.b[1]) : p;
  AuxStream aux;
  bool overlap = knob_i64("GBM_GRM_STD_OVERLAP", 1) != 0 && g.persist && !g.sb.fuse && g.sb.n >= 2 && h < p &&
                 standardize_fits_beside_tiles(n);
  if (overlap) {
    rc = aux_stream(s, aux, &overlap);
    if (rc != GBM_OK) return rc;
  }
  if (!overlap) {
    rc = launch_standardize_rows(X, ldx, p, n, Zt, ldz, mean, sd, keep, q, s);
    if (rc != GBM_OK) return rc;
    return launch_grm_syrk(Zt, ldz, p, n, G, ldg, ws, ws_bytes, s);
  }
  const int64_t need = (g.main_doubles + g.edge_doubles + grm_counter_doubles(g)) * (int64_t)sizeof(double);
  if (!ws || ws_bytes < need)
    return fail(GBM_E_ARG, "gbm_dev_standardize_grm_syrk: workspace too small (" + std::to_string(ws_bytes) + " < " +
                               std::to_string(need) + ")");
  int32_t* ctr = reinterpret_cast<int32_t*>((double*)ws + g.main_doubles + g.edge_doubles + grm_second_doubles(g)) - 8;
  const int64_t lim = g.sb.er > 0 ? g.sb.e0 : n;
  GBM_TRY(launch_standardize_rows(X, ldx, h, n, Zt, ldz, mean, sd, keep, q, s));
  GBM_HIP_TRY(hipMemsetAsync(ctr, 0, 16 * sizeof(int32_t), s));
  GBM_HIP_TRY(hipEventRecord(aux.fork, s));
  GBM_HIP_TRY(hipStreamWaitEvent(aux.s, aux.fork, 0));
  GBM_TRY(launch_persist(g, g.sb, 0, 1, Zt, ldz, p, lim, G, ldg, ws, ctr + 8, s));
  GBM_TRY(launch_standardize_rows(X + h * ldx, ldx, p - h, n, Zt + h * ldz, ldz, mean + h, sd + h, keep + h, q, aux.s,
                                  true));
  if (g.sb.er > 0) GBM_TRY(launch_grm_edge(g, Zt, ldz, p, n, G, ldg, ws, 0, aux.s));
  GBM_TRY(launch_persist(g, g.sb, 1, g.sb.n - 1, Zt, ldz, p, lim, G, ldg, ws, ctr, aux.s));
  GBM_HIP_TRY(hipEventRecord(aux.join, aux.s));
  GBM_HIP_TRY(hipStreamWaitEvent(s, aux.join, 0));
  return GBM_OK;
}

int launch_grm_reduce(int64_t n, int64_t p, double* G, int64_t ldg, const void* ws, hipStream_t s, int accum = 0,
                      int32_t* err_out = nullptr) {
  const GrmPlan g = plan(n, p);
  if (g.sb.n == 1 && g.sb.er == 0) return GBM_OK;
  if (!ws) return fail(GBM_E_ARG, "gbm_dev_grm_reduce: workspace required");
  if (g.sb.er > 0 && !g.edge_concurrent) {
    grm_edge_reduce_kernel<<<(unsigned)((n * g.sb.er + 255) / 256), 256, 0, s>>>((const double*)ws + g.sb.eslab_off, n,
                                                                                 g.sb, G, ldg, accum);
    GBM_LAUNCH_CHECK();
  }
  if (g.sb.n == 1 || g.sb.fuse) return GBM_OK;
  if (g.sb.carry && err_out) {
    GBM_HIP_TRY(hipMemcpyAsync(err_out, (const int32_t*)ws + g.ntiles, sizeof(int32_t), hipMemcpyDeviceToDevice, s));
    return GBM_OK;
  }
  if (g.sb.carry) {
    int32_t err = 0;
    GBM_HIP_TRY(hipMemcpyAsync(&err, (const int32_t*)ws + g.ntiles, sizeof(int32_t), hipMemcpyDeviceToHost, s));
    GBM_HIP_TRY(hipStreamSynchronize(s));
    if (err < 0)
      return fail(GBM_E_HIP, "GRM in-order carry accumulation: an inter-workgroup wait timed out (G is invalid)");
    return GBM_OK;
  }
  grm_slab_reduce_kernel<<<(unsigned)g.ntiles, 256, 0, s>>>((const double*)ws, g.ntiles, g.sb.n, G, ldg, accum);
  GBM_LAUNCH_CHECK();
  return GBM_OK;
}

int launch_grm(const double* Zt, int64_t ldz, int64_t p, int64_t n, double* G, int64_t ldg, void* ws,
               int64_t ws_bytes, hipStream_t s, int accum, int32_t* err_out) {
  if (accum && !grm_can_accumulate(n, p)) return fail(GBM_E_ARG, "GRM: accumulation needs the slab split");
  int rc = launch_grm_syrk(Zt, ldz, p, n, G, ldg, ws, ws_bytes, s, accum);
  if (rc != GBM_OK) return rc;
  return launch_grm_reduce(n, p, G, ldg, ws, s, accum, err_out);
}

bool grm_can_accumulate(int64_t n, int64_t p) {
  const GrmPlan g = plan(n, p);
  return g.sb.n > 1;
}

}

namespace gbm {
__global__ void __launch_bounds__(256) grm_pack_kernel(const double* __restrict__ G, int64_t ldg,
                                                       double* __restrict__ packed, int unpack) {
  const int64_t t = blockIdx.x;
  int64_t ti, tj;
  tile_of(t, ti, tj);
  double* pt = packed + t * (int64_t)(BT * BT);
  for (int e = threadIdx.x * 2; e < BT * BT; e += 512) {
    const int r = e / BT, c = e % BT;
    double* g = const_cast<double*>(G) + (ti * BT + r) * ldg + tj * BT + c;
    if (unpack)
      *reinterpret_cast<double2*>(g) = *reinterpret_cast<const double2*>(pt + e);
    else
      *reinterpret_cast<double2*>(pt + e) = *reinterpret_cast<const double2*>(g);
  }
}
}

extern "C" int64_t gbm_dev_grm_packed_size(int64_t n) {
  const int64_t nt = gbm::npad_of(n) / gbm::BT;
  return nt * (nt + 1) / 2 * gbm::BT * gbm::BT;
}

extern "C" int gbm_dev_grm_pack(const double* G, int64_t ldg, int64_t n, double* packed, void* stream) {
  if (!G || !packed || n < 1 || ldg < gbm::npad_of(n) || (ldg & 1)) return gbm::fail(GBM_E_ARG, "gbm_dev_grm_pack: bad arguments");
  const int64_t nt = gbm::npad_of(n) / gbm::BT;
  gbm::grm_pack_kernel<<<(unsigned)(nt * (nt + 1) / 2), 256, 0, (hipStream_t)stream>>>(G, ldg, packed, 0);
  GBM_LAUNCH_CHECK();
  return GBM_OK;
}

extern "C" int gbm_dev_grm_unpack(const double* packed, int64_t n, double* G, int64_t ldg, void* stream) {
  if (!G || !packed || n < 1 || ldg < gbm::npad_of(n) || (ldg & 1)) return gbm::fail(GBM_E_ARG, "gbm_dev_grm_unpack: bad arguments");
  const int64_t nt = gbm::npad_of(n) / gbm::BT;
  gbm::grm_pack_kernel<<<(unsigned)(nt * (nt + 1) / 2), 256, 0, (hipStream_t)stream>>>(G, ldg, const_cast<double*>(packed), 1);
  GBM_LAUNCH_CHECK();
  return GBM_OK;
}

extern "C" int64_t gbm_dev_grm_workspace(int64_t n, int64_t p) { return gbm::grm_workspace_bytes(n, p); }

extern "C" int gbm_dev_grm(const double* Zt, int64_t ldz, int64_t p, int64_t n, double* G, int64_t ldg,
                           void* workspace, int64_t ws_bytes, void* stream) {
  return gbm::launch_grm(Zt, ldz, p, n, G, ldg, workspace, ws_bytes, (hipStream_t)stream);
}

extern "C" int gbm_dev_grm_accumulate(const double* Zt, int64_t ldz, int64_t p, int64_t n, double* G, int64_t ldg,
                                      void* workspace, int64_t ws_bytes, void* stream) {
  if (!gbm::grm_can_accumulate(n, p))
    return gbm::fail(GBM_E_ARG, "gbm_dev_grm_accumulate: this (n, p) plans a single loci range (gbm_dev_grm_slices == 1); "
                                "use more loci per call");
  return gbm::launch_grm(Zt, ldz, p, n, G, ldg, workspace, ws_bytes, (hipStream_t)stream, 1);
}

extern "C" int gbm_dev_grm_syrk(const double* Zt, int64_t ldz, int64_t p, int64_t n, double* G, int64_t ldg,
                                void* workspace, int64_t ws_bytes, void* stream) {
  return gbm::launch_grm_syrk(Zt, ldz, p, n, G, ldg, workspace, ws_bytes, (hipStream_t)stream);
}

extern "C" int gbm_dev_standardize_grm_syrk(const double* Xt, int64_t ldx, int64_t p, int64_t n, double* Zt, int64_t ldz,
                                            double* mean, double* sd, int32_t* keep, int64_t* q_dev, double* G,
                                            int64_t ldg, void* workspace, int64_t ws_bytes, void* stream) {
  return gbm::launch_standardize_grm_syrk(Xt, ldx, p, n, Zt, ldz, mean, sd, keep, q_dev, G, ldg, workspace, ws_bytes,
                                          (hipStream_t)stream);
}

extern "C" int gbm_dev_grm_reduce(int64_t n, int64_t p, double* G, int64_t ldg, const void* workspace, void* stream) {
  if (!G || n < 1 || p < 1 || ldg < gbm::npad_of(n)) return gbm::fail(GBM_E_ARG, "gbm_dev_grm_reduce: bad arguments");
// ... 45 lines not shown
```

genomicbreedingmodels.jl_amd/csrc/shard_grm.cpp:

```cpp
#include "fit_ctx.h"

namespace gbm {

using Sched = std::vector<std::pair<int64_t, int64_t>>;


int ensure_copy_stream(FitCtx& c) {
  if (!c.copy.s) {
    c.copy.dev = c.dev;
    int lo = 0, hi = 0;
    GBM_HIP_TRY(hipDeviceGetStreamPriorityRange(&lo, &hi));
    GBM_HIP_TRY(hipStreamCreateWithPriority(&c.copy.s, hipStreamNonBlocking, hi));
  }
  return GBM_OK;
}

static int ensure_events(FitCtx& c, int64_t k) {
  while ((int64_t)c.ev.size() < k) {
    hipEvent_t e;
    GBM_HIP_TRY(hipEventCreateWithFlags(&e, hipEventDisableTiming));
    c.ev.push_back(e);
  }
  return GBM_OK;
}
// ... 55 lines not shown
  if (k == 0) return launch_grm(Z, npad, pc, n, (double*)c.G.p, gdim, c.wsg.p, wsb, s, 0, err);
  if (grm_can_accumulate(n, pc)) return launch_grm(Z, npad, pc, n, (double*)c.G.p, gdim, c.wsg.p, wsb, s, 1, err);
  GBM_TRY(launch_grm(Z, npad, pc, n, (double*)c.Gc.p, gdim, c.wsg.p, wsb, s, 0, err));
  return launch_add_inplace((double*)c.G.p, (const double*)c.Gc.p, gdim * gdim, s);
}

static int standardize_chunk(const Problem& pr, FitCtx& c, int64_t j, int64_t pc, double* Zb, int64_t* q) {
  const int64_t n = pr.n, npad = npad_of(n);
  hipStream_t s = c.stream.s;
  if (pr.src == Source::F64) {
    if (npad > n) GBM_HIP_TRY(hipMemset2DAsync(Zb + n, npad * 8, 0, (npad - n) * 8, pc, s));
    return gbm_dev_standardize(Zb, npad, pc, n, Zb, npad, (double*)c.mean.p + j, (double*)c.sd.p + j,
                               (int32_t*)c.keep.p + j, q, s);
  }
  const int ploidy = pr.src == Source::SYNTH ? 2 : pr.ploidy;
  return launch_standardize_i8((const int8_t*)c.D8.p + j * n, n, pc, n, ploidy, Zb, npad, (double*)c.mean.p + j,
                               (double*)c.sd.p + j, (int32_t*)c.keep.p + j, q, s);
}

static int pack_fail(hipError_t e) {
  return fail(GBM_E_HIP, std::string("host-pack upload: HIP error '") + hipGetErrorString(e) + "'");
}

static int packed_upload(const Problem& pr, Shard& sh, const Sched& sched, int slots, int64_t nev, int threads,
                         const std::function<int(int64_t)>& queued) {
  FitCtx& c = sh.x();
  const int64_t n = pr.n;
  int64_t pmax = 0;
  for (const auto& jc : sched) pmax = std::max(pmax, jc.second);
  GBM_TRY(ensure_copy_stream(c));
  GBM_TRY(ensure_pinned(c.pack, slots * pmax * n));
  GBM_TRY(ensure_events(c, nev));
  int rc = GBM_OK;
  {
    ChunkPacker packer(pr.X + sh.j0 * pr.ld, pr.ld, n, sched, static_cast<int8_t*>(c.pack.p), pmax * n, slots, threads);
    for (int64_t k = 0; k < (int64_t)sched.size() && rc == GBM_OK; k++) {
      const int8_t* src = packer.wait(k);
      if (!src) {
        rc = kNotDosage;
        break;
      }
      const int64_t j = sched[k].first, pc = sched[k].second;
      hipError_t e = hipMemcpyAsync((int8_t*)c.D8.p + j * n, src, pc * n, hipMemcpyHostToDevice, c.copy.s);
      if (e == hipSuccess) e = hipEventRecord(c.ev[k % nev], c.copy.s);
      if (e != hipSuccess) rc = pack_fail(e);
      if (rc == GBM_OK && queued) rc = queued(k);
      if (rc == GBM_OK && k >= 1 && (e = hipEventSynchronize(c.ev[(k - 1) % nev])) != hipSuccess) rc = pack_fail(e);
      if (rc == GBM_OK) packer.release_upto(k);
    }
  }
  GBM_HIP_TRY(hipStreamSynchronize(c.copy.s));
  return rc;
}

int prepare_shard(const Problem& pr, Shard& sh, bool center_only, bool sync) {
  FitCtx& c = sh.x();
  const int64_t n = pr.n, npad = npad_of(n), pl = sh.p;
  GBM_HIP_TRY(hipSetDevice(c.dev));
  hipStream_t s = c.stream.s;
  GBM_TRY(ensure(c.Xt, c.dev, pl * npad * 8));
  GBM_TRY(ensure_locus_stats(c, pl));
  if (pr.src == Source::F64) {
    GBM_HIP_TRY(hipMemcpy2DAsync(c.Xt.p, npad * 8, pr.X + sh.j0 * pr.ld, pr.ld * 8, n * 8, pl, hipMemcpyHostToDevice, s));
    if (npad > n) GBM_HIP_TRY(hipMemset2DAsync((double*)c.Xt.p + n, npad * 8, 0, (npad - n) * 8, pl, s));
  } else if (pr.src == Source::SYNTH) {
    GBM_TRY(gbm_dev_synth_genotypes((double*)c.Xt.p, npad, pl, n, pr.seed, sh.j0, s));
  } else {
    GBM_TRY(ensure(c.D8, c.dev, pl * n));
    GBM_HIP_TRY(hipMemcpy2DAsync(c.D8.p, n, pr.D + sh.j0 * pr.ld, pr.ld, n, pl, hipMemcpyHostToDevice, s));
    GBM_TRY(gbm_dev_expand_dosage_i8((const int8_t*)c.D8.p, n, n, pl, pr.ploidy, (double*)c.Xt.p, npad, s));
  }
  GBM_HIP_TRY(hipMemsetAsync(c.q.p, 0, 8, s));
  if (center_only)
    GBM_TRY(launch_center_columns((const double*)c.Xt.p, npad, pl, n, (double*)c.Xt.p, npad, (double*)c.mean.p,
                                  (double*)c.sd.p, (int32_t*)c.keep.p, (int64_t*)c.q.p, s));
  else
    GBM_TRY(gbm_dev_standardize((const double*)c.Xt.p, npad, pl, n, (double*)c.Xt.p, npad, (double*)c.mean.p,
                                (double*)c.sd.p, (int32_t*)c.keep.p, (int64_t*)c.q.p, s));
  GBM_HIP_TRY(hipMemcpyAsync(&sh.q_host, c.q.p, 8, hipMemcpyDeviceToHost, s));
  if (sync) GBM_HIP_TRY(hipStreamSynchronize(s));
  return GBM_OK;
}

int grm_shard(const Problem& pr, Shard& sh) {
  FitCtx& c = sh.x();
  const int64_t n = pr.n, npad = npad_of(n), gdim = gdim_of(n);
  GBM_HIP_TRY(hipSetDevice(c.dev));
  GBM_TRY(ensure(c.G, c.dev, gdim * gdim * 8));
  const int64_t wsb = gbm_dev_grm_workspace(n, sh.p);
  GBM_TRY(ensure(c.wsg, c.dev, wsb));
  return gbm_dev_grm((const double*)c.Xt.p, npad, sh.p, n, (double*)c.G.p, gdim, c.wsg.p, wsb, c.stream.s);
}

int prepare_grm_shard(const Problem& pr, Shard& sh) {
  GBM_TRY(prepare_shard(pr, sh, false, false));
  GBM_TRY(grm_shard(pr, sh));
  GBM_HIP_TRY(hipStreamSynchronize(sh.x().stream.s));
  return GBM_OK;
}

int upload_grm_pipelined(const Problem& pr, Shard& sh, int64_t chunk) {
  FitCtx& c = sh.x();
  const int64_t n = pr.n, npad = npad_of(n), pl = sh.p;
  GBM_HIP_TRY(hipSetDevice(c.dev));
  hipStream_t s = c.stream.s;
  GBM_TRY(ensure_copy_stream(c));
  const Sched sched = shard_schedule(pr, pl, chunk);
  const int64_t nch = (int64_t)sched.size();
  GBM_TRY(ensure_events(c, nch));
  GBM_TRY(ensure(c.Xt, c.dev, pl * npad * 8));
  GBM_TRY(ensure_locus_stats(c, pl));
  if (pr.src == Source::I8) GBM_TRY(ensure(c.D8, c.dev, pl * n));
  int64_t wsb = 0;
  GBM_TRY(ensure_chunked_grm(c, n, sched, &wsb));
  GBM_HIP_TRY(hipMemsetAsync(c.q.p, 0, 8, s));
  double* Xt = (double*)c.Xt.p;
  for (int64_t k = 0; k < nch; k++) {
    const int64_t j = sched[k].first, pc = sched[k].second;
    if (pr.src == Source::F64)
      GBM_HIP_TRY(hipMemcpy2DAsync(Xt + j * npad, npad * 8, pr.X + (sh.j0 + j) * pr.ld, pr.ld * 8, n * 8, pc,
                                   hipMemcpyHostToDevice, c.copy.s));
    else
      GBM_HIP_TRY(hipMemcpy2DAsync((int8_t*)c.D8.p + j * n, n, pr.D + (sh.j0 + j) * pr.ld, pr.ld, n, pc,
                                   hipMemcpyHostToDevice, c.copy.s));
    GBM_HIP_TRY(hipEventRecord(c.ev[k], c.copy.s));
    GBM_HIP_TRY(hipStreamWaitEvent(s, c.ev[k], 0));
    GBM_TRY(standardize_chunk(pr, c, j, pc, Xt + j * npad, (int64_t*)c.q.p));
    GBM_TRY(add_chunk_grm(c, Xt + j * npad, pc, n, k, wsb, nullptr));
  }
  GBM_HIP_TRY(hipMemcpyAsync(&sh.q_host, c.q.p, 8, hipMemcpyDeviceToHost, s));
  GBM_HIP_TRY(hipStreamSynchronize(s));
  return GBM_OK;
}

int upload_grm_pipelined_packed(const Problem& pr, Shard& sh, int64_t chunk, int threads) {
  FitCtx& c = sh.x();
  const int64_t n = pr.n, npad = npad_of(n), pl = sh.p;
  GBM_HIP_TRY(hipSetDevice(c.dev));
  hipStream_t s = c.stream.s;
  const Sched sched = shard_schedule(pr, pl, chunk);
  GBM_TRY(ensure(c.Xt, c.dev, pl * npad * 8));
  GBM_TRY(ensure(c.D8, c.dev, pl * n));
  GBM_TRY(ensure_locus_stats(c, pl));
  int64_t wsb = 0;
  GBM_TRY(ensure_chunked_grm(c, n, sched, &wsb));
  GBM_HIP_TRY(hipMemsetAsync(c.q.p, 0, 8, s));
  double* Xt = (double*)c.Xt.p;
  const int rc = packed_upload(pr, sh, sched, 3, (int64_t)sched.size(), threads, [&](int64_t k) -> int {
    const int64_t j = sched[k].first, pc = sched[k].second;
    const hipError_t e = hipStreamWaitEvent(s, c.ev[k], 0);
    if (e != hipSuccess) return pack_fail(e);
    GBM_TRY(launch_standardize_i8((const int8_t*)c.D8.p + j * n, n, pc, n, 2, Xt + j * npad, npad, (double*)c.mean.p + j,
                                  (double*)c.sd.p + j, (int32_t*)c.keep.p + j, (int64_t*)c.q.p, s));
    return add_chunk_grm(c, Xt + j * npad, pc, n, k, wsb, nullptr);
  });
  if (rc == kNotDosage) GBM_HIP_TRY(hipStreamSynchronize(s));
  GBM_TRY(rc);
  GBM_HIP_TRY(hipMemcpyAsync(&sh.q_host, c.q.p, 8, hipMemcpyDeviceToHost, s));
  GBM_HIP_TRY(hipStreamSynchronize(s));
  return GBM_OK;
}


int plan_streaming(const Problem& pr, Shards& shards, bool reml) {
  const int64_t forced = knob_i64("GBM_STREAM_CHUNK", -1);
  const int64_t n = pr.n, npad = npad_of(n), gdim = gdim_of(n);
  const bool bytes = pr.src != Source::F64;
  if (forced >= 0) {
    for (auto& sh : shards) sh->stream = (forced > 0 && forced < sh->p) ? forced : 0;
    return GBM_OK;
  }
  std::map<int, std::vector<Shard*>> bydev;
  for (auto& sh : shards) bydev[sh->x().dev].push_back(sh.get());
  for (auto& dv : bydev) {
    const int dev = dv.first;
    std::vector<Shard*>& v = dv.second;
    GBM_HIP_TRY(hipSetDevice(dev));
    int64_t held = 0, fixed = 0, resident = 0, dosage = 0, pmax = 0;
    for (Shard* sh : v) {
// ... 209 lines not shown
```

genomicbreedingmodels.jl_amd/gbm/_lib.py:

```python
from __future__ import annotations

import ctypes
import os
import threading

import numpy as np

ABI_VERSION = 212
GBM_OK = 0
GBM_E_ARG = -1
GBM_E_NOTPD = -2
GBM_E_HIP = -3
GBM_E_RCCL = -4
GBM_E_OOM = -5
GBM_E_NODEV = -6
GBM_E_DATA = -7

LIB_PATH = os.environ.get("GBM_LIBGBM") or os.path.join(os.path.dirname(os.path.abspath(__file__)), "libgbm.so")

EXPORTS = (
    "gbm_version", "gbm_last_error", "gbm_device_count", "gbm_device_allocations", "gbm_release_device_cache",
    "gbm_gblup_fit", "gbm_gblup_fit_reml", "gbm_gblup_fit_dosage_i8", "gbm_gblup_fit_synthetic", "gbm_grm", "gbm_grm_ploidy_aware", "gbm_colstats", "gbm_predict",
    "gbm_dev_npad", "gbm_dev_gdim", "gbm_dev_grm_workspace", "gbm_dev_solve_workspace",
    "gbm_dev_synth_genotypes", "gbm_dev_expand_dosage_i8", "gbm_dev_standardize", "gbm_dev_grm",
    "gbm_dev_grm_syrk", "gbm_dev_grm_reduce", "gbm_dev_grm_slices",
    "gbm_dev_gblup_solve", "gbm_dev_marker_effects",
    "gbm_dev_standardize_gather", "gbm_dev_gblup_terms",
    "gbm_session_create", "gbm_session_create_dosage_i8", "gbm_session_create_synthetic", "gbm_session_destroy", "gbm_session_gblup_fit",
    "gbm_session_predict", "gbm_session_reml_objective", "gbm_session_reml", "gbm_session_stats",
    "gbm_session_ridge_path", "gbm_session_ridge_lambda_max", "gbm_brr_fit", "gbm_bayes_fit",
    "gbm_dev_chol_prepare", "gbm_dev_chol_prepare_cols", "gbm_dev_chol_group_size", "gbm_dev_chol_group", "gbm_dev_chol_factor_diag",
    "gbm_dev_chol_strip_doubles", "gbm_dev_chol_strip_pack", "gbm_dev_chol_strip_unpack", "gbm_dev_chol_finish",
    "gbm_dev_grm_packed_size", "gbm_dev_grm_pack", "gbm_dev_grm_unpack",
    "gbm_debug_brr_stats", "gbm_debug_brr_shape", "gbm_debug_brr_trace", "gbm_debug_chol_flow_trace",
    "gbm_dev_synth_dosage_i8", "gbm_dev_standardize_i8", "gbm_dev_grm_accumulate", "gbm_dev_marker_effects_i8",
    "gbm_debug_oom_retries", "gbm_dev_chol_group_panels", "gbm_dev_chol_group_update", "gbm_dev_chol_strip_unpack_rows", "gbm_dev_chol_lower_copy",
    "gbm_dev_chol_area_doubles", "gbm_dev_chol_area_pack", "gbm_dev_chol_area_unpack",
    "gbm_dev_chol_group_update_cols", "gbm_dev_chol_group_update_tiles", "gbm_dev_grm_exact_workspace", "gbm_dev_grm_exact_i8",
    "gbm_gblup_fit_ex", "gbm_gblup_fit_reml_ex", "gbm_gblup_fit_dosage_i8_ex", "gbm_gblup_fit_synthetic_ex",
    "gbm_session_set_grm_mode", "gbm_session_grm_used", "gbm_debug_rccl_calls", "gbm_debug_xg_choose", "gbm_debug_chol_flow_order",
    "gbm_debug_chol_flow_order_check", "gbm_debug_chol_flow_order_size", "gbm_dev_grm_exact_status", "gbm_debug_set",
    "gbm_dev_whiten_rows", "gbm_session_gwas", "gbm_session_enet_path", "gbm_dev_standardize_grm_syrk",
    "gbm_dev_grm_symmetrize", "gbm_dev_rows_times_sym", "gbm_dev_rows_times_sym_workspace", "gbm_session_pcs",
    "gbm_debug_sym_eig", "gbm_session_pair_scan",
)

GBM_GRM_DEFAULT, GBM_GRM_FP64, GBM_GRM_EXACT, GBM_GRM_AUTO, GBM_GRM_DROPIN = -1, 0, 1, 2, 3
GBM_PCS_GRM, GBM_PCS_REFERENCE = 0, 1
PCS_KINDS = {"grm": GBM_PCS_GRM, "reference": GBM_PCS_REFERENCE}
PAIR_OPS = {"mult": 0, "addnorm": 1, "raise": 2, "square": 3, "invoneplus": 4, "log10epsdivlog10eps": 5}
GRM_MODES = {None: GBM_GRM_DEFAULT, "default": GBM_GRM_DEFAULT, "fp64": GBM_GRM_FP64, "exact": GBM_GRM_EXACT,
             "auto": GBM_GRM_AUTO, "dropin": GBM_GRM_DROPIN}


def grm_mode(mode) -> int:
    if isinstance(mode, int) and mode in GRM_MODES.values():
        return mode
    try:
        return GRM_MODES[mode]
    except (KeyError, TypeError):
        raise ArgumentError(f"grm must be one of 'auto', 'exact', 'fp64', 'dropin' or None, got {mode!r}") from None


class ArgumentError(ValueError):
    """Mirrors Julia's ArgumentError thrown by the reference (e.g. src/prediction.jl:67-112)."""


class GBMError(RuntimeError):
    """Mirrors Julia's ErrorException (e.g. src/linear.jl:235-237, src/prediction.jl:125-127)."""


_lock = threading.Lock()
_lib = None

P = ctypes.c_void_p
I64 = ctypes.c_int64
I32 = ctypes.c_int
D = ctypes.c_double
U64 = ctypes.c_uint64


def _declare(lib):
    lib.gbm_version.restype = I32
    lib.gbm_version.argtypes = []
    lib.gbm_last_error.restype = ctypes.c_char_p
    lib.gbm_last_error.argtypes = []
    lib.gbm_device_count.restype = I32
    lib.gbm_device_count.argtypes = [ctypes.POINTER(I32)]
    lib.gbm_device_allocations.restype = I64
    lib.gbm_device_allocations.argtypes = []
    lib.gbm_release_device_cache.restype = I32
    lib.gbm_release_device_cache.argtypes = []
    lib.gbm_dev_chol_prepare.restype = I32
    lib.gbm_dev_chol_prepare.argtypes = [P, I64, I64, D, P, D, P, I64, I64, P, P, I64, P]
    lib.gbm_dev_chol_prepare_cols.restype = I32
    lib.gbm_dev_chol_prepare_cols.argtypes = [P, I64, I64, D, P, D, P, I64, I64, I32, I32, P, P, I64, P]
    lib.gbm_dev_chol_group_size.restype = I64
    lib.gbm_dev_chol_group_size.argtypes = [I64, I64]
    lib.gbm_dev_chol_group.restype = I32
    lib.gbm_dev_chol_group.argtypes = [P, I64, I64, I64, I32, I32, P, P, I64, P]
    for f in ("gbm_dev_chol_group_panels", "gbm_dev_chol_group_update"):
        getattr(lib, f).restype = I32
        getattr(lib, f).argtypes = [P, I64, I64, I64, I32, I32, P, P, I64, P]
    lib.gbm_dev_chol_group_update_cols.restype = I32
    lib.gbm_dev_chol_group_update_cols.argtypes = [P, I64, I64, I64, I32, I32, I64, I64, P, P, I64, P]
    lib.gbm_dev_chol_group_update_tiles.restype = I32
    lib.gbm_dev_chol_group_update_tiles.argtypes = [P, I64, I64, I64, I32, I32, I64, I64, I64, I64, P, P, I64, P]
    lib.gbm_dev_chol_area_doubles.restype = I64
    lib.gbm_dev_chol_area_doubles.argtypes = [I64, I64, I64, I32]
    lib.gbm_dev_chol_area_pack.restype = I32
    lib.gbm_dev_chol_area_pack.argtypes = [P, I64, I64, I64, I64, I32, I32, P, P]
    lib.gbm_dev_chol_area_unpack.restype = I32
    lib.gbm_dev_chol_area_unpack.argtypes = [P, I64, I64, I64, I64, I32, P, P]
    lib.gbm_dev_chol_strip_unpack_rows.restype = I32
    lib.gbm_dev_chol_strip_unpack_rows.argtypes = [P, I64, I64, I64, I64, I32, I32, P, P]
    lib.gbm_dev_chol_lower_copy.restype = I32
    lib.gbm_dev_chol_lower_copy.argtypes = [P, I64, I64, I64, I64, I32, I32, P]
    lib.gbm_dev_chol_factor_diag.restype = I32
    lib.gbm_dev_chol_factor_diag.argtypes = [P, I64, I64, I64, P, P, I64, P]
    lib.gbm_dev_chol_strip_doubles.restype = I64
    lib.gbm_dev_chol_strip_doubles.argtypes = [I64, I64, I64, I32]
    lib.gbm_dev_chol_strip_pack.restype = I32
    lib.gbm_dev_chol_strip_pack.argtypes = [P, I64, I64, I64, I64, I32, I32, P, P]
    lib.gbm_dev_chol_strip_unpack.restype = I32
    lib.gbm_dev_chol_strip_unpack.argtypes = [P, I64, I64, I64, I64, I32, P, P]
    lib.gbm_dev_chol_finish.restype = I32
    lib.gbm_dev_chol_finish.argtypes = [P, I64, I64, P, I64, I64, D, P, P, I64, P, P, P, I64, P]
    lib.gbm_gblup_fit.restype = I32
    lib.gbm_gblup_fit.argtypes = [P, I64, I64, I64, P, I64, I64, D, P, I32, P, P, P, P]
    lib.gbm_gblup_fit_reml.restype = I32
    lib.gbm_gblup_fit_reml.argtypes = [P, I64, I64, I64, P, I64, I64, P, I32, P, P, P, P, P, P, P]
    lib.gbm_gblup_fit_dosage_i8.restype = I32
    lib.gbm_gblup_fit_dosage_i8.argtypes = [P, I64, I64, I64, I32, P, I64, I64, D, P, I32, P, P, P, P]
    lib.gbm_gblup_fit_synthetic.restype = I32
    lib.gbm_gblup_fit_synthetic.argtypes = [U64, I64, I64, P, I64, I64, D, P, I32, P, P, P, P]
    lib.gbm_grm.restype = I32
    lib.gbm_grm.argtypes = [P, I64, I64, I64, P, I32, P, I64, P]
    lib.gbm_grm_ploidy_aware.restype = I32
    lib.gbm_grm_ploidy_aware.argtypes = [P, I64, I64, I64, I32, P, I32, P, I64, P]
    lib.gbm_colstats.restype = I32
    lib.gbm_colstats.argtypes = [P, I64, I64, I64, I32, P, P, P, P]
    lib.gbm_predict.restype = I32
    lib.gbm_predict.argtypes = [P, I64, I64, I64, P, I64, I64, I32, P, I64]
    for f in ("gbm_dev_npad", "gbm_dev_gdim"):
        getattr(lib, f).restype = I64
        getattr(lib, f).argtypes = [I64]
    for f in ("gbm_dev_grm_workspace", "gbm_dev_solve_workspace"):
        getattr(lib, f).restype = I64
        getattr(lib, f).argtypes = [I64, I64]
    lib.gbm_dev_synth_genotypes.restype = I32
    lib.gbm_dev_synth_genotypes.argtypes = [P, I64, I64, I64, U64, I64, P]
    lib.gbm_dev_expand_dosage_i8.restype = I32
    lib.gbm_dev_expand_dosage_i8.argtypes = [P, I64, I64, I64, I32, P, I64, P]
    lib.gbm_dev_standardize.restype = I32
    lib.gbm_dev_standardize.argtypes = [P, I64, I64, I64, P, I64, P, P, P, P, P]
    lib.gbm_dev_synth_dosage_i8.restype = I32
    lib.gbm_dev_synth_dosage_i8.argtypes = [P, I64, I64, I64, U64, I64, P]
    lib.gbm_dev_standardize_i8.restype = I32
    lib.gbm_dev_standardize_i8.argtypes = [P, I64, I64, I64, I32, P, I64, P, P, P, P, P]
    lib.gbm_dev_marker_effects_i8.restype = I32
    lib.gbm_dev_grm_exact_workspace.restype = I64
    lib.gbm_dev_grm_exact_workspace.argtypes = [I64, I64]
    lib.gbm_dev_grm_exact_i8.restype = I32
    lib.gbm_dev_grm_exact_i8.argtypes = [P, I64, I64, I64, I32, P, I64, P, P, P, P, I32, P, I64, P, P]
    lib.gbm_dev_marker_effects_i8.argtypes = [P, I64, I64, I64, I32, P, I64, I64, D, P, P, P, P, P, I64, P, P]
    for f in ("gbm_dev_grm", "gbm_dev_grm_syrk", "gbm_dev_grm_accumulate"):
        getattr(lib, f).restype = I32
        getattr(lib, f).argtypes = [P, I64, I64, I64, P, I64, P, I64, P]
    lib.gbm_dev_standardize_grm_syrk.restype = I32
    lib.gbm_dev_standardize_grm_syrk.argtypes = [P, I64, I64, I64, P, I64, P, P, P, P, P, I64, P, I64, P]
    lib.gbm_dev_grm_reduce.restype = I32
    lib.gbm_dev_grm_reduce.argtypes = [I64, I64, P, I64, P, P]
    lib.gbm_dev_grm_slices.restype = I32
    lib.gbm_dev_grm_slices.argtypes = [I64, I64]
    lib.gbm_dev_gblup_solve.restype = I32
    lib.gbm_dev_gblup_solve.argtypes = [P, I64, I64, D, P, D, P, I64, I64, P, P, I64, P, P, P, I64, P]
    lib.gbm_dev_marker_effects.restype = I32
    lib.gbm_dev_marker_effects.argtypes = [P, I64, I64, I64, P, I64, I64, D, P, P, P, P, P, I64, P, P]
    lib.gbm_dev_standardize_gather.restype = I32
    lib.gbm_dev_standardize_gather.argtypes = [P, I64, I64, P, I64, P, I64, P, P, P, P, I32, P]
    lib.gbm_dev_gblup_terms.restype = I32
    lib.gbm_dev_gblup_terms.argtypes = [P, I64, I64, I64, P, P, P]
    lib.gbm_session_create.restype = I32
    lib.gbm_session_create.argtypes = [P, I64, I64, I64, I32, ctypes.POINTER(P)]
    lib.gbm_session_create_synthetic.restype = I32
    lib.gbm_session_create_synthetic.argtypes = [U64, I64, I64, I32, ctypes.POINTER(P)]
    lib.gbm_session_create_dosage_i8.restype = I32
    lib.gbm_session_create_dosage_i8.argtypes = [P, I64, I64, I64, I32, I32, ctypes.POINTER(P)]
    lib.gbm_session_destroy.restype = None
    lib.gbm_session_destroy.argtypes = [P]
    lib.gbm_session_gblup_fit.restype = I32
    lib.gbm_session_gblup_fit.argtypes = [P, P, I64, P, I64, I64, D, P, P, P, P]
    lib.gbm_session_predict.restype = I32
    lib.gbm_session_predict.argtypes = [P, P, I64, P, I64, I64, P, I64]
    lib.gbm_session_reml_objective.restype = I32
    lib.gbm_session_reml_objective.argtypes = [P, P, I64, P, P, P, I64, P]
    lib.gbm_session_reml.restype = I32
    lib.gbm_session_reml.argtypes = [P, P, I64, P, P, P, P, P]
    lib.gbm_session_ridge_path.restype = I32
    lib.gbm_session_ridge_path.argtypes = [P, P, I64, P, P, I64, P, P, I64, P]
    lib.gbm_session_enet_path.restype = I32
    lib.gbm_session_enet_path.argtypes = [P, P, I64, P, D, P, I64, D, I64, D, D, P, P, I64, P, P, P, P, P]
    lib.gbm_session_ridge_lambda_max.restype = I32
    lib.gbm_session_ridge_lambda_max.argtypes = [P, P, I64, P, P]
    lib.gbm_dev_grm_packed_size.restype = I64
    lib.gbm_dev_grm_packed_size.argtypes = [I64]
    lib.gbm_dev_grm_pack.restype = I32
    lib.gbm_dev_grm_pack.argtypes = [P, I64, I64, P, P]
    lib.gbm_dev_grm_unpack.restype = I32
    lib.gbm_dev_grm_unpack.argtypes = [P, I64, P, I64, P]
    lib.gbm_brr_fit.restype = I32
    lib.gbm_brr_fit.argtypes = [P, I64, I64, I64, P, I64, I64, I64, D, D, U64, I32, P, P, P]
    lib.gbm_bayes_fit.restype = I32
    lib.gbm_bayes_fit.argtypes = [I32, P, I64, I64, I64, P, I64, I64, I64, D, D, D, D, U64, I32, P, P, P, P]
    lib.gbm_debug_oom_retries.restype = I32
    lib.gbm_debug_oom_retries.argtypes = [P, P]
    lib.gbm_session_stats.restype = I32
    lib.gbm_session_stats.argtypes = [P, P, P]
    lib.gbm_gblup_fit_ex.restype = I32
    lib.gbm_gblup_fit_ex.argtypes = [P, I64, I64, I64, P, I64, I64, D, P, I32, I32, P, P, P, P, P]
    lib.gbm_gblup_fit_reml_ex.restype = I32
    lib.gbm_gblup_fit_reml_ex.argtypes = [P, I64, I64, I64, P, I64, I64, P, I32, I32, P, P, P, P, P, P, P, P]
    lib.gbm_gblup_fit_dosage_i8_ex.restype = I32
    lib.gbm_gblup_fit_dosage_i8_ex.argtypes = [P, I64, I64, I64, I32, P, I64, I64, D, P, I32, I32, P, P, P, P, P]
    lib.gbm_gblup_fit_synthetic_ex.restype = I32
    lib.gbm_gblup_fit_synthetic_ex.argtypes = [U64, I64, I64, P, I64, I64, D, P, I32, I32, P, P, P, P, P]
    lib.gbm_session_set_grm_mode.restype = I32
    lib.gbm_session_set_grm_mode.argtypes = [P, I32]
    lib.gbm_session_grm_used.restype = I32
    lib.gbm_session_grm_used.argtypes = [P, P]
    lib.gbm_debug_rccl_calls.restype = I32
    lib.gbm_debug_rccl_calls.argtypes = [P, P]
    lib.gbm_debug_xg_choose.restype = I32
    lib.gbm_debug_xg_choose.argtypes = [D, D, P, P]
    lib.gbm_debug_chol_flow_order.restype = I64
    lib.gbm_debug_chol_flow_order.argtypes = [I32, P, I64]
    lib.gbm_debug_chol_flow_order_size.restype = I64
    lib.gbm_debug_chol_flow_order_size.argtypes = [I32]
    lib.gbm_debug_chol_flow_order_check.restype = I64
    lib.gbm_debug_chol_flow_order_check.argtypes = [I32, P, I64]
    lib.gbm_dev_grm_exact_status.restype = I32
    lib.gbm_dev_grm_exact_status.argtypes = [P, I64, I64, P]
    lib.gbm_dev_whiten_rows.restype = I32
    lib.gbm_dev_whiten_rows.argtypes = [P, I64, I64, P, P, I64, I64, P]
    lib.gbm_session_gwas.restype = I32
    lib.gbm_session_gwas.argtypes = [P, P, I64, P, P, I64, I64, I32, D, D, P, P, P, P]
    lib.gbm_dev_grm_symmetrize.restype = I32
    lib.gbm_dev_grm_symmetrize.argtypes = [P, I64, I64, D, P, I64, P]
    lib.gbm_dev_rows_times_sym_workspace.restype = I64
    lib.gbm_dev_rows_times_sym_workspace.argtypes = [I64, I64]
    lib.gbm_dev_rows_times_sym.restype = I32
    lib.gbm_dev_rows_times_sym.argtypes = [P, I64, I64, P, I64, I64, P, I64, P, I64, P]
    lib.gbm_session_pcs.restype = I32
    lib.gbm_session_pcs.argtypes = [P, P, I64, I32, I64, D, I64, P, P, P, P, P]
    lib.gbm_session_pair_scan.restype = I32
    lib.gbm_session_pair_scan.argtypes = [P, P, I64, P, P, I64, I32, D, I32, D, I32, I64, I64, P, P, P, P, P, P]
    lib.gbm_debug_sym_eig.restype = I32
    lib.gbm_debug_sym_eig.argtypes = [P, I32, P, P]
    lib.gbm_debug_set.restype = I32
# ... 66 lines not shown
```

genomicbreedingmodels.jl_amd/gbm/sharded.py:

```python
from __future__ import annotations

import ctypes

import numpy as np

from . import _lib


class TorchComm:

    def __init__(self, force: bool = False):
        import torch.distributed as dist
        self.dist = dist
        self.world_size = dist.get_world_size() if dist.is_initialized() else 1
        self.rank = dist.get_rank() if dist.is_initialized() else 0
        self.force = bool(force) and dist.is_initialized()

    def all_reduce_sum(self, t):
        if self.world_size > 1 or self.force:
            self.dist.all_reduce(t, op=self.dist.ReduceOp.SUM)

    def all_gather(self, t):
        import torch
        out = torch.empty(self.world_size * t.numel(), dtype=t.dtype, device=t.device)
# ... 129 lines not shown
            for st in stages:
                st.join()
            pending = False
        elif stale:
            exchange(kb, g, "area")
        if not ahead:
            for st, r in zip(stages, ranks):
                st.chol_group_panels(kb, r, nranks)
            exchange(kb, g, "rows")
        ahead = False
        k1 = kb + g
        next_dist = k1 < nb and distributable(k1)
        if overlap and next_dist:
            g1 = int(lib.gbm_dev_chol_group_size(n, k1))
            area_hi = 64 * (k1 + g1)
            for st in stages:
                st.fork()
            if lookahead:
                with stages[0].side():
                    for st, r in zip(stages, ranks):
                        st.chol_group_update_tiles(kb, r, nranks, 64 * k1, area_hi, 64 * k1, gdim)
                    exchange(k1, g1, "area")
                    for st, r in zip(stages, ranks):
                        st.chol_group_panels(k1, r, nranks)
                    exchange(k1, g1, "rows_deferred" if defer_lower else "rows")
                    if defer_lower:
                        for st in stages:
                            st.lower_fork()
                        with stages[0].lower():
                            for st, r in zip(stages, ranks):
                                st.chol_lower_copy(k1, g1, r, nranks)
                for st, r in zip(stages, ranks):
                    st.chol_group_update_tiles(kb, r, nranks, area_hi, gdim, area_hi, gdim)
                ahead = True
            else:
                with stages[0].side():
                    for st, r in zip(stages, ranks):
                        st.chol_group_update_cols(kb, r, nranks, 64 * k1, area_hi)
                    exchange(k1, g1, "area")
                for st, r in zip(stages, ranks):
                    st.chol_group_update_cols(kb, r, nranks, area_hi, gdim)
            pending = True
        else:
            for st, r in zip(stages, ranks):
                st.chol_group_update(kb, r, nranks)
        stale = True
        kb = k1
        if kb >= nb:
            break
        dist = next_dist
        if not dist:
            exchange(kb, nb - kb, "rest")
    for st in stages:
        if defer_lower:
            st.lower_join()
        st.chol_finish()


def assemble_b_hat(mu, msum, B_shards, p_total):
    t = len(mu)
    b_hat = np.zeros((p_total + 1, t))
    b_hat[0] = np.asarray(mu) - np.asarray(msum)
    off = 0
    for B in B_shards:
        b_hat[1 + off:1 + off + B.shape[1]] = B.T
        off += B.shape[1]
    return b_hat


def _written_by_standardize(name):
    attr = "_" + name

    def get(self):
        if self._std_pending:
            self._standardize_now()
        return getattr(self, attr)

    def put(self, value):
        setattr(self, attr, value)

    return property(get, put)


class HipShardStages:

    def __init__(self, n: int, p_local: int, nrhs: int = 1, lambda_: float = 1.0, device: int = 0):
        import torch
        self.torch = torch
        self.lib = _lib.load()
        self.n, self.p, self.nrhs, self.lam = n, p_local, nrhs, float(lambda_)
        self.dev = torch.device("cuda", device)
        lib = self.lib
        self.npad = lib.gbm_dev_npad(n)
        self.gdim = lib.gbm_dev_gdim(n)
        f64 = dict(dtype=torch.float64, device=self.dev)
        self._alloc_rows(f64)
        self.mean = torch.empty(p_local, **f64)
        self.sd = torch.empty(p_local, **f64)
        self.keep = torch.empty(p_local, dtype=torch.int32, device=self.dev)
        self.q = torch.zeros(1, dtype=torch.int64, device=self.dev)
        self.G = torch.empty((self.gdim, self.gdim), **f64)
        self.ws_grm_bytes = self._grm_workspace()
        self.ws_grm = torch.empty(max(self.ws_grm_bytes, 16), dtype=torch.uint8, device=self.dev)
        self.Y = torch.zeros((nrhs, self.npad), **f64)
        self.A = torch.zeros((nrhs, self.npad), **f64)
        self.ws_solve_bytes = lib.gbm_dev_solve_workspace(n, nrhs)
        self.ws_solve = torch.empty(max(self.ws_solve_bytes, 16), dtype=torch.uint8, device=self.dev)
        shapes = [("B", (nrhs, p_local)), ("gebv", (nrhs, self.npad)), ("mu", (nrhs,)), ("msum", (nrhs,))]
        nout = sum(int(np.prod(sh)) for _, sh in shapes) + 1
        self.out = torch.zeros(nout, **f64)
        self.h_out = torch.empty(nout, dtype=torch.float64, pin_memory=True)
        off = 0
        for name, sh in shapes:
            k = int(np.prod(sh))
            setattr(self, name, self.out[off:off + k].view(sh))
            setattr(self, "h_" + name, self.h_out[off:off + k].view(sh))
            off += k
        self.info = self.out[off:].view(torch.int32)[:1]
        self.h_info = self.h_out[off:].view(torch.int32)[:1]

    def _alloc_rows(self, f64):
        self.X = self.torch.empty((self.p, self.npad), **f64)
        self.Z = self.torch.empty((self.p, self.npad), **f64)

    def _grm_workspace(self):
        return self.lib.gbm_dev_grm_workspace(self.n, self.p)

    @staticmethod
    def _p(t):
        return ctypes.c_void_p(t.data_ptr())

    def _stream(self):
        return ctypes.c_void_p(self.torch.cuda.current_stream(self.dev).cuda_stream)

    def generate(self, seed: int, j0: int):
        _lib.check(self.lib.gbm_dev_synth_genotypes(self._p(self.X), self.npad, self.p, self.n, seed, j0,
                                                     self._stream()), "synth")

    def upload_genotypes(self, X_host_colmajor: np.ndarray):
        t = self.torch.from_numpy(np.ascontiguousarray(np.asarray(X_host_colmajor, dtype=np.float64).T))
        self.X.zero_()
        self.X[:, :self.n].copy_(t)

    def load_phenotypes(self, Y: np.ndarray):
        Y = np.asarray(Y, dtype=np.float64)
        if Y.ndim == 1:
            Y = Y[:, None]
        self.Y.zero_()
        self.Y[:, :self.n].copy_(self.torch.from_numpy(np.ascontiguousarray(Y.T)))

    _std_pending = False
    Z = _written_by_standardize("Z")
    mean = _written_by_standardize("mean")
    sd = _written_by_standardize("sd")
    keep = _written_by_standardize("keep")
    q = _written_by_standardize("q")

    def standardize(self):
        self._q.zero_()
        self._std_pending = True

    def _standardize_now(self):
        self._std_pending = False
        _lib.check(self.lib.gbm_dev_standardize(self._p(self.X), self.npad, self.p, self.n, self._p(self._Z), self.npad,
                                                self._p(self._mean), self._p(self._sd), self._p(self._keep),
                                                self._p(self._q), self._stream()), "standardize")

    def grm_syrk(self):
        if self._std_pending:
            self._std_pending = False
            _lib.check(self.lib.gbm_dev_standardize_grm_syrk(
                self._p(self.X), self.npad, self.p, self.n, self._p(self._Z), self.npad, self._p(self._mean),
                self._p(self._sd), self._p(self._keep), self._p(self._q), self._p(self.G), self.gdim,
                self._p(self.ws_grm), self.ws_grm_bytes, self._stream()), "standardize_grm_syrk")
            return
        _lib.check(self.lib.gbm_dev_grm_syrk(self._p(self.Z), self.npad, self.p, self.n, self._p(self.G), self.gdim,
                                             self._p(self.ws_grm), self.ws_grm_bytes, self._stream()), "grm_syrk")

    def grm_reduce(self):
        _lib.check(self.lib.gbm_dev_grm_reduce(self.n, self.p, self._p(self.G), self.gdim, self._p(self.ws_grm),
                                               self._stream()), "grm_reduce")

    def grm_rows(self):
        return self.G[: self.npad]

    def grm_pack(self):
        if getattr(self, "Gp", None) is None:
            self.Gp = self.torch.empty(self.lib.gbm_dev_grm_packed_size(self.n) + 1, dtype=self.torch.float64,
                                       device=self.dev)
        _lib.check(self.lib.gbm_dev_grm_pack(self._p(self.G), self.gdim, self.n, self._p(self.Gp), self._stream()),
                   "grm_pack")
        self.Gp[-1:].copy_(self.q)
        return self.Gp

    def grm_unpack(self):
        _lib.check(self.lib.gbm_dev_grm_unpack(self._p(self.Gp), self.n, self._p(self.G), self.gdim, self._stream()),
                   "grm_unpack")
        self.q.copy_(self.Gp[-1:])

    def solve(self):
        _lib.check(self.lib.gbm_dev_gblup_solve(self._p(self.G), self.gdim, self.n, 0.0, self._p(self.q), self.lam,
                                                self._p(self.Y), self.npad, self.nrhs, self._p(self.A),
                                                self._p(self.gebv), self.npad, self._p(self.mu), self._p(self.info),
                                                self._p(self.ws_solve), self.ws_solve_bytes, self._stream()), "solve")

    def chol_prepare(self):
        _lib.check(self.lib.gbm_dev_chol_prepare(self._p(self.G), self.gdim, self.n, 0.0, self._p(self.q), self.lam,
                                                 self._p(self.Y), self.npad, self.nrhs, self._p(self.info),
                                                 self._p(self.ws_solve), self.ws_solve_bytes, self._stream()),
                   "chol_prepare")

    def chol_prepare_cols(self, rank: int, nranks: int):
        _lib.check(self.lib.gbm_dev_chol_prepare_cols(self._p(self.G), self.gdim, self.n, 0.0, self._p(self.q),
                                                      self.lam, self._p(self.Y), self.npad, self.nrhs, rank, nranks,
                                                      self._p(self.info), self._p(self.ws_solve), self.ws_solve_bytes,
                                                      self._stream()), "chol_prepare_cols")

    def chol_group(self, kb: int, rank: int, nranks: int):
        _lib.check(self.lib.gbm_dev_chol_group(self._p(self.G), self.gdim, self.n, kb, rank, nranks, self._p(self.info),
                                               self._p(self.ws_solve), self.ws_solve_bytes, self._stream()),
                   "chol_group")

    def chol_group_panels(self, kb: int, rank: int, nranks: int):
        _lib.check(self.lib.gbm_dev_chol_group_panels(self._p(self.G), self.gdim, self.n, kb, rank, nranks,
                                                      self._p(self.info), self._p(self.ws_solve), self.ws_solve_bytes,
                                                      self._stream()), "chol_group_panels")

    def chol_group_update_cols(self, kb: int, rank: int, nranks: int, col_lo: int, col_hi: int):
        _lib.check(self.lib.gbm_dev_chol_group_update_cols(self._p(self.G), self.gdim, self.n, kb, rank, nranks, col_lo,
                                                           col_hi, self._p(self.info), self._p(self.ws_solve),
                                                           self.ws_solve_bytes, self._stream()), "chol_group_update_cols")

    def chol_group_update_tiles(self, kb: int, rank: int, nranks: int, row_lo: int, row_hi: int, col_lo: int,
                                col_hi: int):
        _lib.check(self.lib.gbm_dev_chol_group_update_tiles(self._p(self.G), self.gdim, self.n, kb, rank, nranks,
                                                            row_lo, row_hi, col_lo, col_hi, self._p(self.info),
                                                            self._p(self.ws_solve), self.ws_solve_bytes,
                                                            self._stream()), "chol_group_update_tiles")

    def _side_stream(self):
        s = _SIDE_STREAMS.get(self.dev)
        if s is None:
            s = _SIDE_STREAMS[self.dev] = self.torch.cuda.Stream(self.dev, priority=-1)
        return s

    def fork(self):
        self._side_stream().wait_stream(self.torch.cuda.current_stream(self.dev))

    def side(self):
        return self.torch.cuda.stream(self._side_stream())

    def join(self):
        self.torch.cuda.current_stream(self.dev).wait_stream(self._side_stream())

    def _lower_stream(self):
        s = _LOWER_STREAMS.get(self.dev)
        if s is None:
            s = _LOWER_STREAMS[self.dev] = self.torch.cuda.Stream(self.dev)
        return s

    def lower_fork(self):
        self._lower_stream().wait_stream(self.torch.cuda.current_stream(self.dev))

    def lower(self):
        return self.torch.cuda.stream(self._lower_stream())

    def lower_join(self):
        self.torch.cuda.current_stream(self.dev).wait_stream(self._lower_stream())

    def chol_lower_copy(self, kb: int, rows64: int, rank: int, nranks: int):
        _lib.check(self.lib.gbm_dev_chol_lower_copy(self._p(self.G), self.gdim, self.n, kb, rows64, rank, nranks,
                                                    self._stream()), "chol_lower_copy")

    def chol_group_update(self, kb: int, rank: int, nranks: int):
        _lib.check(self.lib.gbm_dev_chol_group_update(self._p(self.G), self.gdim, self.n, kb, rank, nranks,
                                                      self._p(self.info), self._p(self.ws_solve), self.ws_solve_bytes,
                                                      self._stream()), "chol_group_update")

    def area_pack(self, kb: int, rows64: int, rank: int, nranks: int):
        cnt = int(self.lib.gbm_dev_chol_area_doubles(self.n, kb, rows64, nranks))
        buf = self.torch.empty(max(cnt, 1), dtype=self.torch.float64, device=self.dev)[:cnt]
        _lib.check(self.lib.gbm_dev_chol_area_pack(self._p(self.G), self.gdim, self.n, kb, rows64, rank, nranks,
                                                   self._p(buf), self._stream()), "area_pack")
# ... 159 lines not shown
```

include/gbm.h:

```cpp
#ifndef GBM_H
#define GBM_H

#include <stdint.h>

#ifdef __cplusplus
extern "C" {
#endif

#define GBM_VERSION 212

#define GBM_OK 0
#define GBM_E_ARG (-1)
#define GBM_E_NOTPD (-2)
#define GBM_E_HIP (-3)
#define GBM_E_RCCL (-4)
#define GBM_E_OOM (-5)
#define GBM_E_NODEV (-6)
#define GBM_E_DATA (-7)

#define GBM_GRM_DEFAULT (-1)
#define GBM_GRM_FP64 0
#define GBM_GRM_EXACT 1
#define GBM_GRM_AUTO 2
#define GBM_GRM_DROPIN 3
// ... 25 lines not shown
                       double* b_hat_out, double* y_pred_out, double* mu_out, int64_t* q_out,
                       double* lambda_out, double* sigma2_e_out, double* sigma2_u_out);
int gbm_gblup_fit_reml_ex(const double* X, int64_t n, int64_t p, int64_t ldx,
                          const double* Y, int64_t ldy, int64_t nrhs,
                          const int* devices, int ndev, int grm_mode,
                          double* b_hat_out, double* y_pred_out, double* mu_out, int64_t* q_out,
                          double* lambda_out, double* sigma2_e_out, double* sigma2_u_out, int* grm_used_out);

int gbm_gblup_fit_dosage_i8(const int8_t* D, int64_t n, int64_t p, int64_t ldd, int ploidy,
                            const double* Y, int64_t ldy, int64_t nrhs, double lambda,
                            const int* devices, int ndev,
                            double* b_hat_out, double* y_pred_out, double* mu_out, int64_t* q_out);
int gbm_gblup_fit_dosage_i8_ex(const int8_t* D, int64_t n, int64_t p, int64_t ldd, int ploidy,
                               const double* Y, int64_t ldy, int64_t nrhs, double lambda,
                               const int* devices, int ndev, int grm_mode,
                               double* b_hat_out, double* y_pred_out, double* mu_out, int64_t* q_out,
                               int* grm_used_out);

int gbm_gblup_fit_synthetic(uint64_t seed, int64_t n, int64_t p,
                            const double* Y, int64_t ldy, int64_t nrhs, double lambda,
                            const int* devices, int ndev,
                            double* b_hat_out, double* y_pred_out, double* mu_out, int64_t* q_out);
int gbm_gblup_fit_synthetic_ex(uint64_t seed, int64_t n, int64_t p,
                               const double* Y, int64_t ldy, int64_t nrhs, double lambda,
                               const int* devices, int ndev, int grm_mode,
                               double* b_hat_out, double* y_pred_out, double* mu_out, int64_t* q_out,
                               int* grm_used_out);

int gbm_grm(const double* X, int64_t n, int64_t p, int64_t ldx, const int* devices, int ndev,
            double* G_out, int64_t ldg, int64_t* q_out);

int gbm_grm_ploidy_aware(const double* X, int64_t n, int64_t p, int64_t ldx, int ploidy,
                         const int* devices, int ndev, double* G_out, int64_t ldg, double* denom_out);

int gbm_colstats(const double* X, int64_t n, int64_t p, int64_t ldx, int device,
                 double* mean_out, double* sd_out, uint8_t* keep_out, int64_t* q_out);

int gbm_predict(const double* X, int64_t n, int64_t p, int64_t ldx,
                const double* b_hat, int64_t ldb, int64_t nrhs, int device,
                double* out, int64_t ldo);


int64_t gbm_dev_npad(int64_t n);
int64_t gbm_dev_gdim(int64_t n);
int64_t gbm_dev_grm_workspace(int64_t n, int64_t p);
int64_t gbm_dev_solve_workspace(int64_t n, int64_t nrhs);

int gbm_dev_synth_genotypes(double* Xt, int64_t ldx, int64_t p, int64_t n, uint64_t seed,
                            int64_t j0, void* stream);

int gbm_dev_synth_dosage_i8(int8_t* D, int64_t ldd, int64_t p, int64_t n, uint64_t seed, int64_t j0,
                            void* stream);

int gbm_dev_expand_dosage_i8(const int8_t* D, int64_t ldd, int64_t n, int64_t p, int ploidy,
                             double* Xt, int64_t ldx, void* stream);

int gbm_dev_standardize(const double* Xt, int64_t ldx, int64_t p, int64_t n, double* Zt, int64_t ldz,
                        double* mean, double* sd, int32_t* keep, int64_t* q_dev, void* stream);
int gbm_dev_standardize_i8(const int8_t* D, int64_t ldd, int64_t p, int64_t n, int ploidy, double* Zt, int64_t ldz,
                           double* mean, double* sd, int32_t* keep, int64_t* q_dev, void* stream);
int gbm_dev_standardize_gather(const double* Xt, int64_t ldx, int64_t p, const int32_t* idx, int64_t n,
                               double* Zt, int64_t ldz, double* mean, double* sd, int32_t* keep,
                               int64_t* q_dev, int center_only, void* stream);

int gbm_dev_grm(const double* Zt, int64_t ldz, int64_t p, int64_t n, double* G, int64_t ldg,
                void* workspace, int64_t ws_bytes, void* stream);
int gbm_dev_grm_accumulate(const double* Zt, int64_t ldz, int64_t p, int64_t n, double* G, int64_t ldg,
                           void* workspace, int64_t ws_bytes, void* stream);
int gbm_dev_grm_syrk(const double* Zt, int64_t ldz, int64_t p, int64_t n, double* G, int64_t ldg,
                     void* workspace, int64_t ws_bytes, void* stream);
int gbm_dev_grm_reduce(int64_t n, int64_t p, double* G, int64_t ldg, const void* workspace, void* stream);
int gbm_dev_standardize_grm_syrk(const double* Xt, int64_t ldx, int64_t p, int64_t n, double* Zt, int64_t ldz,
                                 double* mean, double* sd, int32_t* keep, int64_t* q_dev, double* G, int64_t ldg,
                                 void* workspace, int64_t ws_bytes, void* stream);
int64_t gbm_dev_grm_packed_size(int64_t n);
int gbm_dev_grm_pack(const double* G, int64_t ldg, int64_t n, double* packed, void* stream);
int gbm_dev_grm_unpack(const double* packed, int64_t n, double* G, int64_t ldg, void* stream);
int gbm_dev_grm_slices(int64_t n, int64_t p);

int gbm_dev_gblup_solve(double* G, int64_t ldg, int64_t n, double inv_q, const int64_t* q_dev, double lambda,
                        const double* Y, int64_t ldy, int64_t nrhs,
                        double* A_out, double* gebv, int64_t lda, double* mu, int32_t* info,
                        void* workspace, int64_t ws_bytes, void* stream);

int gbm_dev_chol_prepare(double* G, int64_t ldg, int64_t n, double inv_q, const int64_t* q_dev, double lambda,
                         const double* Y, int64_t ldy, int64_t nrhs, int32_t* info, void* workspace,
                         int64_t ws_bytes, void* stream);
int gbm_dev_chol_prepare_cols(double* G, int64_t ldg, int64_t n, double inv_q, const int64_t* q_dev, double lambda,
                              const double* Y, int64_t ldy, int64_t nrhs, int rank, int nranks, int32_t* info,
                              void* workspace, int64_t ws_bytes, void* stream);
int64_t gbm_dev_chol_group_size(int64_t n, int64_t kb);
int gbm_dev_chol_group(double* G, int64_t ldg, int64_t n, int64_t kb, int rank, int nranks, int32_t* info,
                       void* workspace, int64_t ws_bytes, void* stream);
int gbm_dev_chol_group_panels(double* G, int64_t ldg, int64_t n, int64_t kb, int rank, int nranks, int32_t* info,
                              void* workspace, int64_t ws_bytes, void* stream);
int gbm_dev_chol_group_update(double* G, int64_t ldg, int64_t n, int64_t kb, int rank, int nranks, int32_t* info,
                              void* workspace, int64_t ws_bytes, void* stream);
int gbm_dev_chol_group_update_cols(double* G, int64_t ldg, int64_t n, int64_t kb, int rank, int nranks,
                                   int64_t col_lo, int64_t col_hi, int32_t* info, void* workspace, int64_t ws_bytes,
                                   void* stream);
int gbm_dev_chol_group_update_tiles(double* G, int64_t ldg, int64_t n, int64_t kb, int rank, int nranks,
                                    int64_t row_lo, int64_t row_hi, int64_t col_lo, int64_t col_hi, int32_t* info,
                                    void* workspace, int64_t ws_bytes, void* stream);
int gbm_dev_chol_factor_diag(double* G, int64_t ldg, int64_t n, int64_t kb, int32_t* info, void* workspace,
                             int64_t ws_bytes, void* stream);
int64_t gbm_dev_chol_strip_doubles(int64_t n, int64_t kb, int64_t rows64, int nranks);
int gbm_dev_chol_strip_pack(const double* G, int64_t ldg, int64_t n, int64_t kb, int64_t rows64, int rank,
                            int nranks, double* buf, void* stream);
int gbm_dev_chol_strip_unpack(double* G, int64_t ldg, int64_t n, int64_t kb, int64_t rows64, int nranks,
                              const double* gathered, void* stream);
int64_t gbm_dev_chol_area_doubles(int64_t n, int64_t kb, int64_t rows64, int nranks);
int gbm_dev_chol_area_pack(const double* G, int64_t ldg, int64_t n, int64_t kb, int64_t rows64, int rank,
                           int nranks, double* buf, void* stream);
int gbm_dev_chol_area_unpack(double* G, int64_t ldg, int64_t n, int64_t kb, int64_t rows64, int nranks,
                             const double* gathered, void* stream);
int gbm_dev_chol_lower_copy(double* G, int64_t ldg, int64_t n, int64_t kb, int64_t rows64, int rank, int nranks,
                            void* stream);
int gbm_dev_chol_strip_unpack_rows(double* G, int64_t ldg, int64_t n, int64_t kb, int64_t rows64, int rank,
                                   int nranks, const double* gathered, void* stream);
int gbm_dev_chol_finish(double* G, int64_t ldg, int64_t n, const double* Y, int64_t ldy, int64_t nrhs,
                        double lambda, double* A_out, double* gebv, int64_t lda, double* mu, int32_t* info,
                        void* workspace, int64_t ws_bytes, void* stream);

int gbm_dev_gblup_terms(const double* G, int64_t ldg, int64_t n, int64_t nrhs, const void* workspace,
                        double* terms, void* stream);

int gbm_dev_whiten_rows(const double* G, int64_t ldg, int64_t n, const void* solve_workspace, double* R,
                        int64_t ldr, int64_t rows, void* stream);

int gbm_dev_grm_symmetrize(const double* G, int64_t ldg, int64_t n, double scale, double* K, int64_t ldk,
                           void* stream);

int64_t gbm_dev_rows_times_sym_workspace(int64_t n, int64_t rows);
int gbm_dev_rows_times_sym(const double* K, int64_t ldk, int64_t n, const double* Qt, int64_t ldq, int64_t rows,
                           double* Yt, int64_t ldy, void* workspace, int64_t ws_bytes, void* stream);

int gbm_dev_marker_effects(const double* Zt, int64_t ldz, int64_t p, int64_t n,
                           const double* A, int64_t lda, int64_t nrhs, double inv_q, const int64_t* q_dev,
                           const double* mean, const double* sd, const int32_t* keep,
                           double* B, int64_t ldb, double* msum, void* stream);

int64_t gbm_dev_grm_exact_workspace(int64_t n, int64_t p);
int gbm_dev_grm_exact_i8(const int8_t* D, int64_t ldd, int64_t p, int64_t n, int ploidy, double* G, int64_t ldg,
                         double* mean, double* sd, int32_t* keep, int64_t* q_dev, int accum, void* workspace,
                         int64_t ws_bytes, int32_t* slices_out, void* stream);
int gbm_dev_grm_exact_status(const void* workspace, int64_t n, int64_t p, void* stream);

int gbm_dev_marker_effects_i8(const int8_t* D, int64_t ldd, int64_t p, int64_t n, int ploidy,
                              const double* A, int64_t lda, int64_t nrhs, double inv_q, const int64_t* q_dev,
                              const double* mean, const double* sd, const int32_t* keep,
                              double* B, int64_t ldb, double* msum, void* stream);

typedef struct gbm_session gbm_session;
int gbm_session_create(const double* X, int64_t n, int64_t p, int64_t ldx, int device, gbm_session** out);
int gbm_session_create_dosage_i8(const int8_t* D, int64_t n, int64_t p, int64_t ldd, int ploidy, int device,
                                 gbm_session** out);
int gbm_session_create_synthetic(uint64_t seed, int64_t n, int64_t p, int device, gbm_session** out);
void gbm_session_destroy(gbm_session* s);
int gbm_session_set_grm_mode(gbm_session* s, int grm_mode);
int gbm_session_grm_used(gbm_session* s, int* grm_used);
int gbm_session_gblup_fit(gbm_session* s, const int64_t* idx, int64_t n_train, const double* Y, int64_t ldy,
                          int64_t nrhs, double lambda, double* b_hat_out, double* y_pred_out, double* mu_out,
                          int64_t* q_out);
int gbm_session_predict(gbm_session* s, const int64_t* idx, int64_t n_val, const double* b_hat, int64_t ldb,
                        int64_t nrhs, double* out, int64_t ldo);
int gbm_session_reml_objective(gbm_session* s, const int64_t* idx, int64_t n_train, const double* y,
// ... 70 lines not shown
```

Measured before the change: 12.13 billion.

## Fold GRM slab reduction into solve prepare and fuse back-solve finish kernels

Defers the GRM slab reduction on single-shard non-REML fits and runs it inside the solve's prepare pass: one kernel reduces the slabs, builds the shifted system matrix and zeroes the flow and back-solve flags. This removes a separate full pass over G and two memsets. The back-solve kernel also gains a fused variant that inverts the diagonal blocks in LDS and computes mu and GEBV inline, replacing the diag-inverse, gls_mu and gebv kernel launches. The cost is more shared memory and register pressure in the back-solve, plus a lazy-reduce mechanism in the Python path to keep G reads correct.

Result: no change. 12.15 billion (median of 6 runs) (+0.2%).

```diff
diff --git a/genomicbreedingmodels.jl_amd/csrc/capi.cpp b/genomicbreedingmodels.jl_amd/csrc/capi.cpp
--- a/genomicbreedingmodels.jl_amd/csrc/capi.cpp
+++ b/genomicbreedingmodels.jl_amd/csrc/capi.cpp
@@ -49,7 +49,12 @@
       const int64_t wss = gbm_dev_solve_workspace(n, nt);
       GBM_TRY(ensure(c.wss, c.dev, wss));
       GBM_HIP_TRY(hipMemcpy2DAsync(c.Y.p, npad * 8, Y + t0 * ldy, ldy * 8, n * 8, nt, hipMemcpyHostToDevice, s));
-      if (!distributed)
+      if (sh.reduce_due) {
+        sh.reduce_due = false;
+        GBM_TRY(gbm_dev_grm_reduce_gblup_solve(n, sh.p, (double*)c.G.p, gdim, c.wsg.p, inv_q, nullptr, lambda,
+                                               (const double*)c.Y.p, npad, nt, (double*)c.A.p, (double*)c.gebv.p, npad,
+                                               (double*)c.mu.p, (int32_t*)c.info.p, c.wss.p, wss, s));
+      } else if (!distributed)
         GBM_TRY(gbm_dev_gblup_solve((double*)c.G.p, gdim, n, inv_q, nullptr, lambda, (const double*)c.Y.p, npad, nt,
                                     (double*)c.A.p, (double*)c.gebv.p, npad, (double*)c.mu.p, (int32_t*)c.info.p,
                                     c.wss.p, wss, s));
@@ -187,7 +192,7 @@
         }
         return upload_grm_pipelined(pr, sh, chunk);
       }
-      return prepare_grm_shard(pr, sh);
+      return prepare_grm_shard(pr, sh, shards.size() == 1 && !reml && !force_rccl() && knob_i64("GBM_SOLVE_FOLD", 1) != 0);
     });
   };
   {
diff --git a/genomicbreedingmodels.jl_amd/csrc/chol.hip b/genomicbreedingmodels.jl_amd/csrc/chol.hip
--- a/genomicbreedingmodels.jl_amd/csrc/chol.hip
+++ b/genomicbreedingmodels.jl_amd/csrc/chol.hip
@@ -18,7 +18,7 @@
 int64_t chol_flow_flag_bytes(int64_t gdim);
 bool chol_flow_enabled(int64_t npad);
 int launch_chol_flow(double* G, int64_t ldg, int64_t gdim, double* Ld, double* Dinv, void* flag_block, int32_t* info,
-                     hipStream_t s);
+                     hipStream_t s, bool flags_clear = false);
 
 __global__ void __launch_bounds__(256) prepare_v_kernel(double* __restrict__ G, int64_t ld, int64_t n,
                                                         int64_t npad, int64_t gdim, double inv_q,
@@ -436,11 +436,22 @@
 
 constexpr int RC = 4;
 
+struct FinishArgs {
+  const double* Ld;
+  double* Linv;
+  const double* Y;
+  int64_t ldy, n, npad;
+  double* mu;
+  double* gebv;
+  double lambda;
+};
+template <bool FUSED>
 __global__ void __launch_bounds__(256) back_solve_kernel(const double* __restrict__ G, int64_t ld,
-                                                         const double* __restrict__ Linv, int64_t nb,
+                                                         const double* Linv, int64_t nb,
                                                          const double* __restrict__ W, double* A,
                                                          int64_t lda, int64_t nrhs, int32_t* __restrict__ flags,
-                                                         int32_t* __restrict__ info) {
+                                                         int32_t* __restrict__ info, FinishArgs f) {
+  __shared__ double Ub[FUSED ? 2 * NB * (NB + 1) : 1];
   __shared__ double part[4][RC][NB];
   __shared__ double rl[RC][NB];
   __shared__ double ah[RC][NB];
@@ -454,16 +465,55 @@
   const __amdgpu_buffer_rsrc_t rA =
       __builtin_amdgcn_make_buffer_rsrc(A, (short)0, (int)(a_bytes < 0x7fffffff ? a_bytes : 0x7fffffff), 0x00020000);
   double uh[16], ul[16], lb[16];
-#pragma unroll
-  for (int jj = 0; jj < 16; jj++) {
-    uh[jj] = Linv[(h0 + lane) * NB + j0 + jj];
-    ul[jj] = lo ? Linv[(l0 + lane) * NB + j0 + jj] : 0.0;
-    lb[jj] = lo ? G[(h0 + j0 + jj) * ld + l0 + lane] : 0.0;
+  if constexpr (FUSED) {
+    constexpr int UP = NB + 1;
+    for (int r = wave; r < (lo ? 2 * NB : NB); r += 4)
+      Ub[r * UP + lane] = f.Ld[((r < NB ? h0 : l0 - NB) + r) * NB + lane];
+    if (blockIdx.x == 0)
+      for (int64_t t = 0; t < nrhs; t++)
+        for (int64_t i = f.npad + tid; i < lda; i += 256) f.gebv[t * lda + i] = 0.0;
+    __syncthreads();
+    if (wave == 0 || (wave == 1 && lo)) {
+      double* U = Ub + wave * NB * UP;
+      const int64_t b0 = wave ? l0 : h0;
+      double x[NB];
+#pragma unroll
+      for (int i = NB - 1; i >= 0; i--) {
+        double p0 = 0.0, p1 = 0.0, p2 = 0.0, p3 = 0.0;
+#pragma unroll
+        for (int k = i + 1; k < NB; k += 4) {
+          p0 = fma(U[i * UP + k], x[k], p0);
+          if (k + 1 < NB) p1 = fma(U[i * UP + k + 1], x[k + 1], p1);
+          if (k + 2 < NB) p2 = fma(U[i * UP + k + 2], x[k + 2], p2);
+          if (k + 3 < NB) p3 = fma(U[i * UP + k + 3], x[k + 3], p3);
+        }
+        x[i] = (i <= lane) ? (((lane == i) ? 1.0 : 0.0) - ((p0 + p1) + (p2 + p3))) * rcp_nr(U[i * UP + i]) : 0.0;
+      }
+#pragma unroll
+      for (int i = 0; i < NB; i++) {
+        f.Linv[(b0 + i) * NB + lane] = x[i];
+        U[i * UP + lane] = x[i];
+      }
+    }
+    __syncthreads();
+#pragma unroll
+    for (int jj = 0; jj < 16; jj++) {
+      uh[jj] = Ub[lane * UP + j0 + jj];
+      ul[jj] = lo ? Ub[(NB + lane) * UP + j0 + jj] : 0.0;
+      lb[jj] = lo ? G[(h0 + j0 + jj) * ld + l0 + lane] : 0.0;
+    }
+  } else {
+#pragma unroll
+    for (int jj = 0; jj < 16; jj++) {
+      uh[jj] = Linv[(h0 + lane) * NB + j0 + jj];
+      ul[jj] = lo ? Linv[(l0 + lane) * NB + j0 + jj] : 0.0;
+      lb[jj] = lo ? G[(h0 + j0 + jj) * ld + l0 + lane] : 0.0;
+    }
   }
   if (tid == 0) ok_s = 1;
   int32_t pass = 0;
   auto solve_block = [&](int64_t b0, const double (&ui)[16], const double (&acc)[RC], const double (&w)[RC], int tc,
-                         int64_t t0, double (*out)[NB]) {
+                         int64_t t0, double (*out)[NB], const double (&y)[RC], const double (&m)[RC]) {
 #pragma unroll
     for (int t = 0; t < RC; t++) part[wave][t][lane] = acc[t];
     lds_sync();
@@ -479,24 +529,52 @@
       part[wave][t][lane] = s;
     }
     lds_sync();
-    if (wave == 0)
-      for (int t = 0; t < tc; t++) {
-        const double v = ((part[0][t][lane] + part[1][t][lane]) + part[2][t][lane]) + part[3][t][lane];
-        st_agent(A + (t0 + t) * lda + b0 + lane, v);
-        if (out) out[t][lane] = v;
-      }
+    if constexpr (FUSED) {
+      if (wave == 0)
+#pragma unroll
+        for (int t = 0; t < RC; t++)
+          if (t < tc) {
+            const double v = ((part[0][t][lane] + part[1][t][lane]) + part[2][t][lane]) + part[3][t][lane];
+            st_agent(A + (t0 + t) * lda + b0 + lane, v);
+            if (out) out[t][lane] = v;
+            f.gebv[(t0 + t) * lda + b0 + lane] = b0 + lane < f.n ? m[t] + (y[t] - m[t]) - f.lambda * v : 0.0;
+          }
+    } else {
+      if (wave == 0)
+        for (int t = 0; t < tc; t++) {
+          const double v = ((part[0][t][lane] + part[1][t][lane]) + part[2][t][lane]) + part[3][t][lane];
+          st_agent(A + (t0 + t) * lda + b0 + lane, v);
+          if (out) out[t][lane] = v;
+        }
+    }
   };
   for (int64_t t0 = 0; t0 < nrhs; t0 += RC) {
     pass++;
     const int tc = (int)(nrhs - t0 < RC ? nrhs - t0 : RC);
     double acch[RC] = {0.0, 0.0, 0.0, 0.0}, accl[RC] = {0.0, 0.0, 0.0, 0.0};
     double wh[RC] = {0.0, 0.0, 0.0, 0.0}, wl[RC] = {0.0, 0.0, 0.0, 0.0};
+    double yh[RC] = {0.0, 0.0, 0.0, 0.0}, yl[RC] = {0.0, 0.0, 0.0, 0.0}, mt[RC] = {0.0, 0.0, 0.0, 0.0};
     if (wave == 0)
 #pragma unroll
       for (int t = 0; t < RC; t++)
         if (t < tc) {
-          wh[t] = W[(t0 + t) * lda + h0 + lane];
-          if (lo) wl[t] = W[(t0 + t) * lda + l0 + lane];
+          if constexpr (FUSED) {
+            const int64_t npad = f.npad;
+            const double c11 = -G[npad * ld + npad];
+            const double c1y = -G[npad * ld + npad + 1 + t0 + t];
+            const double m = c1y / c11;
+            mt[t] = m;
+            if (blockIdx.x == 0 && lane == 0) f.mu[t0 + t] = m;
+            wh[t] = G[(npad + 1 + t0 + t) * ld + h0 + lane] - m * G[npad * ld + h0 + lane];
+            if (h0 + lane < f.n) yh[t] = f.Y[(t0 + t) * f.ldy + h0 + lane];
+            if (lo) {
+              wl[t] = G[(npad + 1 + t0 + t) * ld + l0 + lane] - m * G[npad * ld + l0 + lane];
+              if (l0 + lane < f.n) yl[t] = f.Y[(t0 + t) * f.ldy + l0 + lane];
+            }
+          } else {
+            wh[t] = W[(t0 + t) * lda + h0 + lane];
+            if (lo) wl[t] = W[(t0 + t) * lda + l0 + lane];
+          }
         }
     bool ok = true;
     for (int64_t c = nb - 1; c > bh && ok; c--) {
@@ -527,7 +605,7 @@
       }
     }
     if (!ok) ok_s = 0;
-    solve_block(h0, uh, acch, wh, tc, t0, lo ? ah : nullptr);
+    solve_block(h0, uh, acch, wh, tc, t0, lo ? ah : nullptr, yh, mt);
     publish_flag(&flags[bh], pass, tid);
     if (lo) {
       for (int t = 0; t < tc; t++) {
@@ -537,7 +615,7 @@
         accl[t] += sl;
       }
       lds_sync();
-      solve_block(l0, ul, accl, wl, tc, t0, nullptr);
+      solve_block(l0, ul, accl, wl, tc, t0, nullptr, yl, mt);
       publish_flag(&flags[bl], pass, tid);
     }
     if (!ok_s) return;
@@ -722,15 +800,31 @@
   return 1;
 }
 
+struct GrmFold {
+  int64_t p;
+  const void* ws;
+};
 int solve_prepare(double* G, int64_t ldg, int64_t n, double inv_q, const int64_t* q_dev, double lambda,
                   const double* Y, int64_t ldy, int64_t nrhs, int32_t* info, void* workspace, hipStream_t s,
-                  bool factor_first = true, ColKeep keep = ColKeep{}) {
+                  bool factor_first = true, ColKeep keep = ColKeep{}, const GrmFold* fold = nullptr,
+                  bool zero_flow = false) {
   const int64_t npad = npad_of(n), gdim = gdim_of(n);
   const SolveWs w = solve_ws(workspace, npad);
   chol_refresh_tuning();
-  prepare_v_kernel<<<(unsigned)gdim, 256, 0, s>>>(G, ldg, n, npad, gdim, inv_q, q_dev, lambda, Y, ldy, nrhs, info,
-                                                  keep);
-  GBM_LAUNCH_CHECK();
+  if (fold) {
+    PrepareV pv{n, npad, gdim, inv_q, q_dev, lambda, Y, ldy, nrhs, info, {nullptr, nullptr}, {0, 0}};
+    if (zero_flow) {
+      pv.zero[0] = reinterpret_cast<int32_t*>(w.flow);
+      pv.zero_words[0] = chol_flow_flag_bytes(gdim) / 4;
+    }
+    pv.zero[1] = w.flags;
+    pv.zero_words[1] = npad / NB;
+    GBM_TRY(launch_grm_reduce_prepare(n, fold->p, G, ldg, fold->ws, pv, s));
+  } else {
+    prepare_v_kernel<<<(unsigned)gdim, 256, 0, s>>>(G, ldg, n, npad, gdim, inv_q, q_dev, lambda, Y, ldy, nrhs, info,
+                                                    keep);
+    GBM_LAUNCH_CHECK();
+  }
   if (!factor_first) return GBM_OK;
   factor_diag_kernel<<<1, 256, 0, s>>>(G, ldg, 0, w.Ld, w.Dinv, info);
   GBM_LAUNCH_CHECK();
@@ -827,15 +921,25 @@
 }
 
 int solve_finish(double* G, int64_t ldg, int64_t n, const double* Y, int64_t ldy, int64_t nrhs, double lambda,
-                 double* A_out, double* gebv, int64_t lda, double* mu, int32_t* info, void* workspace, hipStream_t s) {
+                 double* A_out, double* gebv, int64_t lda, double* mu, int32_t* info, void* workspace, hipStream_t s,
+                 bool flags_clear = false) {
   const int64_t npad = npad_of(n), nb = npad / NB;
   const SolveWs w = solve_ws(workspace, npad);
+  if (knob_i64("GBM_SOLVE_FOLD", 1) != 0) {
+    if (!flags_clear) GBM_HIP_TRY(hipMemsetAsync(w.flags, 0, (size_t)nb * sizeof(int32_t), s));
+    const FinishArgs f{w.Ld, w.Linv, Y, ldy, n, npad, mu, gebv, lambda};
+    back_solve_kernel<true><<<(unsigned)((nb + 1) / 2), 256, 0, s>>>(G, ldg, w.Linv, nb, nullptr, A_out, lda, nrhs,
+                                                                     w.flags, info, f);
+    GBM_LAUNCH_CHECK();
+    return GBM_OK;
+  }
   diag_inverse_kernel<<<(unsigned)nb, 64, 0, s>>>(w.Ld, w.Linv);
   GBM_LAUNCH_CHECK();
   const unsigned gx = (unsigned)((lda + 255) / 256 < 1024 ? (lda + 255) / 256 : 1024);
   gls_mu_kernel<<<dim3(gx, (unsigned)nrhs), 256, 0, s>>>(G, ldg, npad, nrhs, gebv, lda, mu, w.flags);
   GBM_LAUNCH_CHECK();
-  back_solve_kernel<<<(unsigned)((nb + 1) / 2), 256, 0, s>>>(G, ldg, w.Linv, nb, gebv, A_out, lda, nrhs, w.flags, info);
+  back_solve_kernel<false><<<(unsigned)((nb + 1) / 2), 256, 0, s>>>(G, ldg, w.Linv, nb, gebv, A_out, lda, nrhs, w.flags,
+                                                                    info, FinishArgs{});
   GBM_LAUNCH_CHECK();
   gebv_kernel<<<dim3(gx, (unsigned)nrhs), 256, 0, s>>>(Y, ldy, n, A_out, gebv, lda, mu, lambda);
   GBM_LAUNCH_CHECK();
@@ -853,31 +957,56 @@
 
 }
 
-extern "C" int gbm_dev_gblup_solve(double* G, int64_t ldg, int64_t n, double inv_q, const int64_t* q_dev,
-                                   double lambda, const double* Y, int64_t ldy, int64_t nrhs, double* A_out,
-                                   double* gebv, int64_t lda, double* mu, int32_t* info, void* workspace,
-                                   int64_t ws_bytes, void* stream) {
+namespace {
+int gblup_solve(double* G, int64_t ldg, int64_t n, double inv_q, const int64_t* q_dev, double lambda, const double* Y,
+                int64_t ldy, int64_t nrhs, double* A_out, double* gebv, int64_t lda, double* mu, int32_t* info,
+                void* workspace, int64_t ws_bytes, hipStream_t s, const GrmFold* fold) {
   const int64_t npad = npad_of(n);
   if (!Y || !A_out || !gebv || !mu || ldy < n || lda < npad || nrhs < 1 || nrhs > MAXRHS || !(lambda > 0.0) ||
       !(q_dev || inv_q > 0.0))
     return fail(GBM_E_ARG, "gbm_dev_gblup_solve: bad arguments (need ldg >= gdim(n), lda >= npad(n), "
                            "1 <= nrhs <= 63, lambda > 0, inv_q > 0)");
   GBM_TRY(check_solve_args(G, ldg, n, info, workspace, ws_bytes, "gbm_dev_gblup_solve"));
-  hipStream_t s = (hipStream_t)stream;
   if (chol_flow_enabled(npad)) {
-    GBM_TRY(solve_prepare(G, ldg, n, inv_q, q_dev, lambda, Y, ldy, nrhs, info, workspace, s, false));
+    GBM_TRY(solve_prepare(G, ldg, n, inv_q, q_dev, lambda, Y, ldy, nrhs, info, workspace, s, false, ColKeep{}, fold,
+                          fold != nullptr));
     const SolveWs w = solve_ws(workspace, npad);
-    GBM_TRY(launch_chol_flow(G, ldg, gdim_of(n), w.Ld, w.Dinv, w.flow, info, s));
-    return solve_finish(G, ldg, n, Y, ldy, nrhs, lambda, A_out, gebv, lda, mu, info, workspace, s);
-  }
-  GBM_TRY(solve_prepare(G, ldg, n, inv_q, q_dev, lambda, Y, ldy, nrhs, info, workspace, s));
+    GBM_TRY(launch_chol_flow(G, ldg, gdim_of(n), w.Ld, w.Dinv, w.flow, info, s, fold != nullptr));
+    return solve_finish(G, ldg, n, Y, ldy, nrhs, lambda, A_out, gebv, lda, mu, info, workspace, s, fold != nullptr);
+  }
+  GBM_TRY(solve_prepare(G, ldg, n, inv_q, q_dev, lambda, Y, ldy, nrhs, info, workspace, s, true, ColKeep{}, fold));
   const int64_t nb = npad / NB;
   for (int64_t kb = 0; kb < nb;) {
     int64_t g = 1;
     GBM_TRY(solve_group(G, ldg, n, kb, info, workspace, s, &g));
     kb += g;
   }
-  return solve_finish(G, ldg, n, Y, ldy, nrhs, lambda, A_out, gebv, lda, mu, info, workspace, s);
+  return solve_finish(G, ldg, n, Y, ldy, nrhs, lambda, A_out, gebv, lda, mu, info, workspace, s, fold != nullptr);
+}
+}
+
+extern "C" int gbm_dev_gblup_solve(double* G, int64_t ldg, int64_t n, double inv_q, const int64_t* q_dev,
+                                   double lambda, const double* Y, int64_t ldy, int64_t nrhs, double* A_out,
+                                   double* gebv, int64_t lda, double* mu, int32_t* info, void* workspace,
+                                   int64_t ws_bytes, void* stream) {
+  return gblup_solve(G, ldg, n, inv_q, q_dev, lambda, Y, ldy, nrhs, A_out, gebv, lda, mu, info, workspace, ws_bytes,
+                     (hipStream_t)stream, nullptr);
+}
+
+extern "C" int gbm_dev_grm_reduce_gblup_solve(int64_t n, int64_t p, double* G, int64_t ldg, const void* grm_workspace,
+                                              double inv_q, const int64_t* q_dev, double lambda, const double* Y,
+                                              int64_t ldy, int64_t nrhs, double* A_out, double* gebv, int64_t lda,
+                                              double* mu, int32_t* info, void* workspace, int64_t ws_bytes,
+                                              void* stream) {
+  if (!G || n < 1 || p < 1 || ldg < npad_of(n)) return fail(GBM_E_ARG, "gbm_dev_grm_reduce_gblup_solve: bad arguments");
+  if (knob_i64("GBM_SOLVE_FOLD", 1) != 0 && grm_workspace && grm_reduce_foldable(n, p)) {
+    const GrmFold fold{p, grm_workspace};
+    return gblup_solve(G, ldg, n, inv_q, q_dev, lambda, Y, ldy, nrhs, A_out, gebv, lda, mu, info, workspace, ws_bytes,
+                       (hipStream_t)stream, &fold);
+  }
+  GBM_TRY(gbm_dev_grm_reduce(n, p, G, ldg, grm_workspace, stream));
+  return gbm_dev_gblup_solve(G, ldg, n, inv_q, q_dev, lambda, Y, ldy, nrhs, A_out, gebv, lda, mu, info, workspace,
+                             ws_bytes, stream);
 }
 
 extern "C" int gbm_dev_chol_prepare(double* G, int64_t ldg, int64_t n, double inv_q, const int64_t* q_dev,
diff --git a/genomicbreedingmodels.jl_amd/csrc/chol_flow.hip b/genomicbreedingmodels.jl_amd/csrc/chol_flow.hip
--- a/genomicbreedingmodels.jl_amd/csrc/chol_flow.hip
+++ b/genomicbreedingmodels.jl_amd/csrc/chol_flow.hip
@@ -936,7 +936,7 @@
 }
 
 int launch_chol_flow(double* G, int64_t ldg, int64_t gdim, double* Ld, double* Dinv, void* flag_block, int32_t* info,
-                     hipStream_t s) {
+                     hipStream_t s, bool flags_clear) {
   const int64_t nbc = gdim / FT;
   const int64_t ntasks = nbc * (nbc + 1) / 2;
   if (nbc < 2 || (int64_t)FT * ldg * 8 > 0x7fffffff || nbc * nbc > 0x3fffffff || nbc > 0x7fff)
@@ -944,7 +944,7 @@
   const int32_t* order = nullptr;
   int nwork = 0;
   GBM_TRY(flow_order_dev((int)nbc, &order, &nwork));
-  GBM_HIP_TRY(hipMemsetAsync(flag_block, 0, (size_t)chol_flow_flag_bytes(gdim), s));
+  if (!flags_clear) GBM_HIP_TRY(hipMemsetAsync(flag_block, 0, (size_t)chol_flow_flag_bytes(gdim), s));
   if (::gbm::knob("GBM_TEST_CHOL_FLOW_ABORT")) GBM_HIP_TRY(hipMemsetAsync(info, 0xFF, sizeof(int32_t), s));
   const char* ew = ::gbm::knob("GBM_CHOL_FLOW_WGS");
   const int64_t workers = ew && atoll(ew) > 0 ? atoll(ew) : flow_cus() - 2;
diff --git a/genomicbreedingmodels.jl_amd/csrc/fit_ctx.h b/genomicbreedingmodels.jl_amd/csrc/fit_ctx.h
--- a/genomicbreedingmodels.jl_amd/csrc/fit_ctx.h
+++ b/genomicbreedingmodels.jl_amd/csrc/fit_ctx.h
@@ -41,6 +41,7 @@
   int64_t stream = 0;
   bool exact = false;
   bool d8_ready = false;
+  bool reduce_due = false;
   int leader = -1;
   ~Shard() {
     if (c) pool().release(std::move(c));
@@ -132,8 +133,8 @@
 int ensure_copy_stream(FitCtx& c);
 int64_t host_chunk(int64_t p);
 int prepare_shard(const Problem& pr, Shard& sh, bool center_only = false, bool sync = true);
-int grm_shard(const Problem& pr, Shard& sh);
-int prepare_grm_shard(const Problem& pr, Shard& sh);
+int grm_shard(const Problem& pr, Shard& sh, bool defer_reduce = false);
+int prepare_grm_shard(const Problem& pr, Shard& sh, bool defer_reduce = false);
 int upload_grm_pipelined(const Problem& pr, Shard& sh, int64_t chunk);
 int upload_grm_pipelined_packed(const Problem& pr, Shard& sh, int64_t chunk, int threads);
 int plan_streaming(const Problem& pr, Shards& shards, bool reml);
diff --git a/genomicbreedingmodels.jl_amd/csrc/gbm_internal.h b/genomicbreedingmodels.jl_amd/csrc/gbm_internal.h
--- a/genomicbreedingmodels.jl_amd/csrc/gbm_internal.h
+++ b/genomicbreedingmodels.jl_amd/csrc/gbm_internal.h
@@ -43,6 +43,20 @@
 int launch_grm(const double* Zt, int64_t ldz, int64_t p, int64_t n, double* G, int64_t ldg,
                void* ws, int64_t ws_bytes, hipStream_t s, int accum = 0, int32_t* err_out = nullptr);
 bool grm_can_accumulate(int64_t n, int64_t p);
+struct PrepareV {
+  int64_t n, npad, gdim;
+  double inv_q;
+  const int64_t* q_dev;
+  double lambda;
+  const double* Y;
+  int64_t ldy, nrhs;
+  int32_t* info;
+  int32_t* zero[2];
+  int64_t zero_words[2];
+};
+bool grm_reduce_foldable(int64_t n, int64_t p);
+int launch_grm_reduce_prepare(int64_t n, int64_t p, double* G, int64_t ldg, const void* ws, const PrepareV& pv,
+                              hipStream_t s);
 int launch_standardize_rows(const double* Xt, int64_t ldx, int64_t p, int64_t n, double* Zt, int64_t ldz, double* mean,
                             double* sd, int32_t* keep, int64_t* q_dev, hipStream_t s, bool beside_tiles = false);
 bool standardize_fits_beside_tiles(int64_t n);
diff --git a/genomicbreedingmodels.jl_amd/csrc/grm.hip b/genomicbreedingmodels.jl_amd/csrc/grm.hip
--- a/genomicbreedingmodels.jl_amd/csrc/grm.hip
+++ b/genomicbreedingmodels.jl_amd/csrc/grm.hip
@@ -540,6 +540,65 @@
       acc.y = old.y + acc.y;
     }
     *g = acc;
+  }
+}
+
+__device__ __forceinline__ double prepare_v_value(int64_t i, int64_t j, double g, int64_t n, double inv_q,
+                                                  double lambda) {
+  if (j < i) return 0.0;
+  return (i < n && j < n) ? g * inv_q + (i == j ? lambda : 0.0) : (i == j ? 1.0 : 0.0);
+}
+
+__global__ void __launch_bounds__(256) grm_reduce_prepare_kernel(const double* __restrict__ slab, int64_t ntiles,
+                                                                 int nslices, double* __restrict__ G, int64_t ldg,
+                                                                 int64_t T, PrepareV a) {
+  const double inv_q = a.q_dev ? 1.0 / (double)(*a.q_dev) : a.inv_q;
+  if ((int64_t)blockIdx.x < ntiles) {
+    const int64_t t = blockIdx.x;
+    int64_t ti, tj;
+    tile_of(t, ti, tj);
+    const int64_t per = (int64_t)BT * BT;
+    for (int e = threadIdx.x * 2; e < BT * BT; e += 256 * 2) {
+      double2 acc = make_double2(0.0, 0.0);
+      for (int sl = 0; sl < nslices; sl++) {
+#if GBM_GRM_RED_NT
+        typedef double d2v __attribute__((ext_vector_type(2)));
+        const d2v v = __builtin_nontemporal_load(reinterpret_cast<const d2v*>(slab + ((int64_t)sl * ntiles + t) * per + e));
+#else
+        const double2 v = *reinterpret_cast<const double2*>(slab + ((int64_t)sl * ntiles + t) * per + e);
+#endif
+        acc.x += v.x;
+        acc.y += v.y;
+      }
+      const int64_t i = ti * BT + e / BT, j = tj * BT + e % BT;
+      if (j >= (i / kCholNB) * kCholNB) {
+        acc.x = prepare_v_value(i, j, acc.x, a.n, inv_q, a.lambda);
+        acc.y = prepare_v_value(i, j + 1, acc.y, a.n, inv_q, a.lambda);
+      }
+      *reinterpret_cast<double2*>(G + i * ldg + j) = acc;
+    }
+    return;
+  }
+  const int64_t w = (int64_t)blockIdx.x - ntiles, nw = (int64_t)gridDim.x - ntiles;
+  if (w == 0 && threadIdx.x == 0) *a.info = 0;
+#pragma unroll
+  for (int z = 0; z < 2; z++)
+    for (int64_t k = w * 256 + threadIdx.x; k < a.zero_words[z]; k += nw * 256) a.zero[z][k] = 0;
+  const int lane = threadIdx.x & 63;
+  const int64_t i = w * 4 + (threadIdx.x >> 6);
+  if (i >= a.gdim) return;
+  double* row = G + i * ldg;
+  const int64_t jbeg = (i / kCholNB) * kCholNB;
+  for (int64_t j = (i < T && jbeg < T ? T : jbeg) + lane; j < a.gdim; j += 64) {
+    double v = 0.0;
+    if (i < a.npad) {
+      if (j < a.npad) v = prepare_v_value(i, j, (i < a.n && j < a.n) ? row[j] : 0.0, a.n, inv_q, a.lambda);
+      else if (i < a.n) {
+        const int64_t tt = j - a.npad;
+        v = tt == 0 ? 1.0 : (tt <= a.nrhs ? a.Y[(tt - 1) * a.ldy + i] : 0.0);
+      }
+    }
+    row[j] = v;
   }
 }
 
@@ -1117,6 +1176,30 @@
   return GBM_OK;
 }
 
+bool grm_reduce_foldable(int64_t n, int64_t p) {
+  const GrmPlan g = plan(n, p);
+  return g.persist && g.sb.n > 1 && !g.sb.carry && !g.sb.fuse;
+}
+
+int launch_grm_reduce_prepare(int64_t n, int64_t p, double* G, int64_t ldg, const void* ws, const PrepareV& pv,
+                              hipStream_t s) {
+  const GrmPlan g = plan(n, p);
+  if (!(g.persist && g.sb.n > 1 && !g.sb.carry && !g.sb.fuse) || !ws || pv.n != n || pv.npad != npad_of(n) ||
+      pv.gdim != gdim_of(n) || ldg < pv.gdim)
+    return fail(GBM_E_ARG, "grm_reduce_prepare: not a persistent slab plan (see grm_reduce_foldable)");
+  if (g.sb.er > 0 && !g.edge_concurrent) {
+    grm_edge_reduce_kernel<<<(unsigned)((n * g.sb.er + 255) / 256), 256, 0, s>>>((const double*)ws + g.sb.eslab_off, n,
+                                                                                 g.sb, G, ldg, 0);
+    GBM_LAUNCH_CHECK();
+  }
+  const int64_t T = g.sb.er > 0 ? g.sb.e0 : pv.npad;
+  const int64_t strips = (pv.gdim + 3) / 4;
+  grm_reduce_prepare_kernel<<<(unsigned)(g.ntiles + strips), 256, 0, s>>>((const double*)ws, g.ntiles, g.sb.n, G, ldg,
+                                                                         T, pv);
+  GBM_LAUNCH_CHECK();
+  return GBM_OK;
+}
+
 int launch_grm(const double* Zt, int64_t ldz, int64_t p, int64_t n, double* G, int64_t ldg, void* ws,
                int64_t ws_bytes, hipStream_t s, int accum, int32_t* err_out) {
   if (accum && !grm_can_accumulate(n, p)) return fail(GBM_E_ARG, "GRM: accumulation needs the slab split");
diff --git a/genomicbreedingmodels.jl_amd/csrc/shard_grm.cpp b/genomicbreedingmodels.jl_amd/csrc/shard_grm.cpp
--- a/genomicbreedingmodels.jl_amd/csrc/shard_grm.cpp
+++ b/genomicbreedingmodels.jl_amd/csrc/shard_grm.cpp
@@ -161,19 +161,23 @@
   return GBM_OK;
 }
 
-int grm_shard(const Problem& pr, Shard& sh) {
+int grm_shard(const Problem& pr, Shard& sh, bool defer_reduce) {
   FitCtx& c = sh.x();
   const int64_t n = pr.n, npad = npad_of(n), gdim = gdim_of(n);
   GBM_HIP_TRY(hipSetDevice(c.dev));
   GBM_TRY(ensure(c.G, c.dev, gdim * gdim * 8));
   const int64_t wsb = gbm_dev_grm_workspace(n, sh.p);
   GBM_TRY(ensure(c.wsg, c.dev, wsb));
+  if (defer_reduce) {
+    sh.reduce_due = true;
+    return gbm_dev_grm_syrk((const double*)c.Xt.p, npad, sh.p, n, (double*)c.G.p, gdim, c.wsg.p, wsb, c.stream.s);
+  }
   return gbm_dev_grm((const double*)c.Xt.p, npad, sh.p, n, (double*)c.G.p, gdim, c.wsg.p, wsb, c.stream.s);
 }
 
-int prepare_grm_shard(const Problem& pr, Shard& sh) {
+int prepare_grm_shard(const Problem& pr, Shard& sh, bool defer_reduce) {
   GBM_TRY(prepare_shard(pr, sh, false, false));
-  GBM_TRY(grm_shard(pr, sh));
+  GBM_TRY(grm_shard(pr, sh, defer_reduce));
   GBM_HIP_TRY(hipStreamSynchronize(sh.x().stream.s));
   return GBM_OK;
 }
diff --git a/genomicbreedingmodels.jl_amd/gbm/_lib.py b/genomicbreedingmodels.jl_amd/gbm/_lib.py
--- a/genomicbreedingmodels.jl_amd/gbm/_lib.py
+++ b/genomicbreedingmodels.jl_amd/gbm/_lib.py
@@ -42,7 +42,7 @@
     "gbm_debug_chol_flow_order_check", "gbm_debug_chol_flow_order_size", "gbm_dev_grm_exact_status", "gbm_debug_set",
     "gbm_dev_whiten_rows", "gbm_session_gwas", "gbm_session_enet_path", "gbm_dev_standardize_grm_syrk",
     "gbm_dev_grm_symmetrize", "gbm_dev_rows_times_sym", "gbm_dev_rows_times_sym_workspace", "gbm_session_pcs",
-    "gbm_debug_sym_eig", "gbm_session_pair_scan",
+    "gbm_debug_sym_eig", "gbm_session_pair_scan", "gbm_dev_grm_reduce_gblup_solve",
 )
 
 GBM_GRM_DEFAULT, GBM_GRM_FP64, GBM_GRM_EXACT, GBM_GRM_AUTO, GBM_GRM_DROPIN = -1, 0, 1, 2, 3
@@ -175,6 +175,8 @@
     lib.gbm_dev_grm_slices.argtypes = [I64, I64]
     lib.gbm_dev_gblup_solve.restype = I32
     lib.gbm_dev_gblup_solve.argtypes = [P, I64, I64, D, P, D, P, I64, I64, P, P, I64, P, P, P, I64, P]
+    lib.gbm_dev_grm_reduce_gblup_solve.restype = I32
+    lib.gbm_dev_grm_reduce_gblup_solve.argtypes = [I64, I64, P, I64, P, D, P, D, P, I64, I64, P, P, I64, P, P, P, I64, P]
     lib.gbm_dev_marker_effects.restype = I32
     lib.gbm_dev_marker_effects.argtypes = [P, I64, I64, I64, P, I64, I64, D, P, P, P, P, P, I64, P, P]
     lib.gbm_dev_standardize_gather.restype = I32
diff --git a/genomicbreedingmodels.jl_amd/gbm/sharded.py b/genomicbreedingmodels.jl_amd/gbm/sharded.py
--- a/genomicbreedingmodels.jl_amd/gbm/sharded.py
+++ b/genomicbreedingmodels.jl_amd/gbm/sharded.py
@@ -235,6 +235,19 @@
     return property(get, put)
 
 
+def _written_by_grm_reduce():
+
+    def get(self):
+        if self._reduce_pending:
+            self._reduce_now()
+        return self._G
+
+    def put(self, value):
+        self._G = value
+
+    return property(get, put)
+
+
 class HipShardStages:
 
     def __init__(self, n: int, p_local: int, nrhs: int = 1, lambda_: float = 1.0, device: int = 0):
@@ -330,8 +343,15 @@
         _lib.check(self.lib.gbm_dev_grm_syrk(self._p(self.Z), self.npad, self.p, self.n, self._p(self.G), self.gdim,
                                              self._p(self.ws_grm), self.ws_grm_bytes, self._stream()), "grm_syrk")
 
+    _reduce_pending = False
+    G = _written_by_grm_reduce()
+
     def grm_reduce(self):
-        _lib.check(self.lib.gbm_dev_grm_reduce(self.n, self.p, self._p(self.G), self.gdim, self._p(self.ws_grm),
+        self._reduce_pending = True
+
+    def _reduce_now(self):
+        self._reduce_pending = False
+        _lib.check(self.lib.gbm_dev_grm_reduce(self.n, self.p, self._p(self._G), self.gdim, self._p(self.ws_grm),
                                                self._stream()), "grm_reduce")
 
     def grm_rows(self):
@@ -352,6 +372,13 @@
         self.q.copy_(self.Gp[-1:])
 
     def solve(self):
+        if self._reduce_pending:
+            self._reduce_pending = False
+            _lib.check(self.lib.gbm_dev_grm_reduce_gblup_solve(
+                self.n, self.p, self._p(self._G), self.gdim, self._p(self.ws_grm), 0.0, self._p(self.q), self.lam,
+                self._p(self.Y), self.npad, self.nrhs, self._p(self.A), self._p(self.gebv), self.npad, self._p(self.mu),
+                self._p(self.info), self._p(self.ws_solve), self.ws_solve_bytes, self._stream()), "reduce_solve")
+            return
         _lib.check(self.lib.gbm_dev_gblup_solve(self._p(self.G), self.gdim, self.n, 0.0, self._p(self.q), self.lam,
                                                 self._p(self.Y), self.npad, self.nrhs, self._p(self.A),
                                                 self._p(self.gebv), self.npad, self._p(self.mu), self._p(self.info),
diff --git a/include/gbm.h b/include/gbm.h
--- a/include/gbm.h
+++ b/include/gbm.h
@@ -131,6 +131,10 @@
                         const double* Y, int64_t ldy, int64_t nrhs,
                         double* A_out, double* gebv, int64_t lda, double* mu, int32_t* info,
                         void* workspace, int64_t ws_bytes, void* stream);
+int gbm_dev_grm_reduce_gblup_solve(int64_t n, int64_t p, double* G, int64_t ldg, const void* grm_workspace,
+                                   double inv_q, const int64_t* q_dev, double lambda, const double* Y, int64_t ldy,
+                                   int64_t nrhs, double* A_out, double* gebv, int64_t lda, double* mu, int32_t* info,
+                                   void* workspace, int64_t ws_bytes, void* stream);
 
 int gbm_dev_chol_prepare(double* G, int64_t ldg, int64_t n, double inv_q, const int64_t* q_dev, double lambda,
                          const double* Y, int64_t ldy, int64_t nrhs, int32_t* info, void* workspace,
```
